# OpenResearchInstitute/opv-cxx-demod

Hardware: AMD Instinct MI355X
Metric: IQ Msamples/s demod+Viterbi (×real-time @2.168MSPS); BER vs ref (higher is better)
Workload: dtype f64; 1 GPU; configs[3]: 64 concurrent IQ streams/GPU x 1000 frames, -s semantics, amp 2000, f0 -2000..+2000 Hz across the 64 streams of a shard (SURVEY.md §8d C4: edge streams on the AFC clamp, outside the +/-1530 Hz search span), Eb/N0 16 dB; streams_per_gpu=64, parallelism=streams sharded 64/GPU, no data-path collective

## Files before the change

opv-cxx-demod_amd/csrc/k_frontend.hip:

```cpp
#include <hip/hip_runtime.h>
#include <math.h>

#include <type_traits>

#include "k_frontend_common.h"

namespace {

constexpr uint32_t kTile = OPV_TILE_SAMPLES;
constexpr uint32_t kRing = 2 * kTile;
constexpr uint32_t kRingBytes = kRing * 4;
constexpr uint32_t kGuardBytes = 16;
constexpr uint32_t kBack = 11;
constexpr uint32_t kAhead = 56;
static_assert((kRing & (kRing - 1)) == 0, "ring must be a power of two");

constexpr uint32_t kTabOff = kRingBytes + kGuardBytes;
static_assert(kTabOff % 16 == 0, "16-byte LDS alignment");
constexpr uint32_t kAtanQBytes = 1025 * 32;
constexpr uintptr_t kRbLdsBase = 16;
static_assert(kRbLdsBase + kTabOff + kAtanQBytes == OPV_RB_LDS_I16, "launch size of the int16-ring shape");

constexpr uint32_t kF64Ring = 2048;
constexpr uint32_t kF64RingBytes = kF64Ring * 32;
constexpr uint32_t kF64Chunk = 256;
constexpr uint32_t kF64TabOff = 0;
constexpr uint32_t kF64RingOff = kAtanQBytes;
constexpr uint32_t kF64FlagOff = kF64RingOff + kF64RingBytes;
constexpr uint32_t kF64WaitSpins = 1u << 22;
constexpr uint32_t kHelperSpins = 1u << 22;
static_assert(kRbLdsBase + kF64FlagOff + 16 == OPV_RB_LDS_F64, "launch size of the fp64-ring shape");
static_assert(kF64Ring % kF64Chunk == 0 && (kF64Ring & (kF64Ring - 1)) == 0, "chunks tile the power-of-two ring");

typedef double d2v __attribute__((ext_vector_type(2)));
typedef __attribute__((address_space(3))) unsigned char lbyte;
typedef __attribute__((address_space(3))) int lint;
typedef __attribute__((address_space(3))) double ldouble;
typedef __attribute__((address_space(3))) d2v ld2v;

__device__ inline double swap32_add(double a, double b) {
    auto lo = __builtin_amdgcn_permlane32_swap((unsigned)dlo(a), (unsigned)dlo(b), false, false);
    auto hi = __builtin_amdgcn_permlane32_swap((unsigned)dhi(a), (unsigned)dhi(b), false, false);
    return mkd((int)hi[0], (int)lo[0]) + mkd((int)hi[1], (int)lo[1]);
}
__device__ inline double swap16_add(double a, double b) {
    auto lo = __builtin_amdgcn_permlane16_swap((unsigned)dlo(a), (unsigned)dlo(b), false, false);
    auto hi = __builtin_amdgcn_permlane16_swap((unsigned)dhi(a), (unsigned)dhi(b), false, false);
    return mkd((int)hi[0], (int)lo[0]) + mkd((int)hi[1], (int)lo[1]);
}
template <int N>
__device__ inline double row_bcast(double old, double v) { return __builtin_amdgcn_update_dpp(old, v, 0x150 + N, 0xF, 0xF, false); }
__device__ inline uint32_t uni(uint32_t v) { return (uint32_t)__builtin_amdgcn_readfirstlane((int)v); }
__device__ inline bool uni_lt(double a, double b) { return __builtin_amdgcn_fcmp(a, b, 4 ) != 0ull; }
__device__ inline bool uni_eq(double a, double b) { return __builtin_amdgcn_fcmp(a, b, 1 ) != 0ull; }

struct TagFirst { static constexpr bool first = true, wide = true; };
struct TagSecond { static constexpr bool first = false, wide = true; };
struct TagSteady { static constexpr bool first = false, wide = false; };

struct SinCosK {
    double s0, s1, s2, s3;
    double c0, c1, c2, c3, c4;
};
#define OPV_EXPJ_ASM \
    "v_mul_f64 %[x], %[kfs], %[fo]\n\t" \
    "v_mul_f64 %[u], %[x], %[x]\n\t" \
    "v_fma_f64 %[r], %[c4], %[u], %[c3]\n\t" \
    "v_fma_f64 %[p], %[s3], %[u], %[s2]\n\t" \
    "v_fma_f64 %[r], %[r], %[u], %[c2]\n\t" \
    "v_fma_f64 %[p], %[p], %[u], %[s1]\n\t" \
    "v_fma_f64 %[r], %[r], %[u], %[c1]\n\t" \
    "v_fma_f64 %[p], %[p], %[u], %[s0]\n\t" \
    "v_fma_f64 %[r], %[r], %[u], %[c0]\n\t" \
    "v_mul_f64 %[t], %[x], %[u]\n\t" \
    "v_fma_f64 %[xc], %[r], %[u], 1.0\n\t" \
    "v_fma_f64 %[xs], %[t], %[p], %[x]"
__device__ inline void expj_small(double kfs, double fo, const SinCosK& k, double& xs, double& xc) {
    double x, u, p, r, t;
    asm(OPV_EXPJ_ASM
        : [x] "=&v"(x), [u] "=&v"(u), [p] "=&v"(p), [r] "=&v"(r), [t] "=&v"(t), [xs] "=&v"(xs), [xc] "=&v"(xc)
        : [kfs] "v"(kfs), [fo] "v"(fo), [s0] "v"(k.s0), [s1] "v"(k.s1), [s2] "v"(k.s2), [s3] "v"(k.s3),
          [c0] "v"(k.c0), [c1] "v"(k.c1), [c2] "v"(k.c2), [c3] "v"(k.c3), [c4] "v"(k.c4));
}
__device__ inline void expj_small_clamped(double kfs, double fo_raw, double fo_lo, double fo_hi, const SinCosK& k, double& fo,
                                          double& xs, double& xc) {
    double x, u, p, r, t;
    asm("v_max_f64 %[fo], %[raw], %[lo]\n\t"
        "v_min_f64 %[fo], %[fo], %[hi]\n\t" OPV_EXPJ_ASM
        : [fo] "=&v"(fo), [x] "=&v"(x), [u] "=&v"(u), [p] "=&v"(p), [r] "=&v"(r), [t] "=&v"(t), [xs] "=&v"(xs), [xc] "=&v"(xc)
        : [raw] "v"(fo_raw), [lo] "v"(fo_lo), [hi] "v"(fo_hi), [kfs] "v"(kfs), [s0] "v"(k.s0), [s1] "v"(k.s1), [s2] "v"(k.s2), [s3] "v"(k.s3),
          [c0] "v"(k.c0), [c1] "v"(k.c1), [c2] "v"(k.c2), [c3] "v"(k.c3), [c4] "v"(k.c4));
}
#undef OPV_EXPJ_ASM

}

#include "opv_atan2.h"

typedef __attribute__((address_space(3))) volatile uint32_t lds_flag;
__device__ inline lds_flag* f64_flags(lbyte* lds_all) {
    return reinterpret_cast<lds_flag*>(lds_all + kF64FlagOff);
}

__device__ void f64_ring_helper(const OpvStream& st, lbyte* lds_all) {
    const uint32_t lane = threadIdx.x & 63u;
    lds_flag* const fl = f64_flags(lds_all);
    const uint32_t n_avail = uni((uint32_t)st.n_avail), origin = uni((uint32_t)st.origin);
    const int* const iq = reinterpret_cast<const int*>(st.iq);
    uint32_t fill = ((origin >= kBack ? origin - kBack : 0u) / kF64Chunk) * kF64Chunk;
    const uint32_t fill_end = n_avail + kAhead + 2u;
    uint32_t spins = 0;
    while ((int)(fill - fill_end) < 0) {
        if (fl[2] != 0u) return;
        if ((int)(fl[0] + kF64Ring - fill - kF64Chunk) < 0) {
            if (++spins > kHelperSpins) return;
            __builtin_amdgcn_s_sleep(8);
            continue;
        }
        spins = 0;
        constexpr uint32_t kPerLane = kF64Chunk / 64u;
        const uint32_t n0 = fill + lane;
        int w[kPerLane], wn[kPerLane];
        if (fill + kF64Chunk < n_avail) {
#pragma unroll
            for (uint32_t k = 0; k < kPerLane; ++k) { w[k] = iq[n0 + 64u * k]; wn[k] = iq[n0 + 64u * k + 1u]; }
        } else {
#pragma unroll
            for (uint32_t k = 0; k < kPerLane; ++k) {
                const uint32_t n = n0 + 64u * k;
                w[k] = n < n_avail ? iq[n] : 0;
                wn[k] = n + 1u < n_avail ? iq[n + 1u] : 0;
            }
        }
#pragma unroll
        for (uint32_t k = 0; k < kPerLane; ++k) {
            const int xr = (int)(short)(w[k] & 0xFFFF), xi = w[k] >> 16;
            const int yr = (int)(short)(wn[k] & 0xFFFF) - xr, yi = (wn[k] >> 16) - xi;
            ld2v* e = reinterpret_cast<ld2v*>(lds_all + kF64RingOff + (((n0 + 64u * k) & (kF64Ring - 1u)) << 5));
            e[0] = d2v{(double)xr, (double)xi};
            e[1] = d2v{(double)yr, (double)yi};
        }
        __builtin_amdgcn_fence(__ATOMIC_RELEASE, "workgroup");
        fill += kF64Chunk;
        if (lane == 0u) fl[1] = fill;
    }
}

template <int WPB, bool F64 = false>
__device__ __forceinline__ void msk_frontend_body(OpvStream* __restrict__ streams, OpvGlobalCfg cfg, int n_streams,
                                                  lbyte* lds_all) {
    const int lane = threadIdx.x & 63;
    const int wave = WPB == 1 ? 0 : __builtin_amdgcn_readfirstlane((int)(threadIdx.x >> 6));
    const int sidx = (int)blockIdx.x * WPB + wave;
    const uint64_t dbg_t0 = __builtin_amdgcn_s_memtime(), dbg_r0 = __builtin_amdgcn_s_memrealtime();

    lbyte* const lds = lds_all + (F64 ? kF64RingOff : wave * kTabOff);
    const lbyte* ringb = lds;
    const ldouble* atab = reinterpret_cast<const ldouble*>(lds_all + (F64 ? kF64TabOff : WPB * kTabOff));
    if (sidx >= n_streams) return;
    OpvStream& st = streams[sidx];

    const int jsamp = (lane & 15) == 15 ? 50 : lane - (lane >> 4);
    const double kf = (double)(jsamp - 10);
    const double kfs = kf * kDeltaPerHz;
    double wr[15], wi[15];
    {
        const int row = lane >> 4, t = lane & 15, u = t & 7;
        const bool is_p = u >= 6, imag = t >= 8;
        const int gate = (u < 2 || is_p) ? 1 : ((u & 1) ? 2 : 0);
        const bool tone2 = is_p ? false : (u < 2 ? u == 1 : u >= 4);
#pragma unroll
        for (int n = 0; n < 15; ++n) {
            const int i = 15 * row + n - 10 * gate;
            double sn, cs;
            sincospi((double)i / 80.0, &sn, &cs);
            const bool in = i >= 0 && i < 40;
            const double a = in ? cs : 0.0, b = in ? -sn : 0.0;
            double r_, i_;
            if (is_p) { r_ = (t == 6) ? a : (t == 15 ? b : 0.0); i_ = (t == 7) ? b : (t == 14 ? a : 0.0); }
            else if (!imag) { r_ = a; i_ = tone2 ? -b : b; }
            else { r_ = tone2 ? b : -b; i_ = a; }
            wr[n] = r_; wi[n] = i_;
            asm volatile("" : "+v"(wr[n]), "+v"(wi[n]));
        }
    }
    SinCosK sck;
    sck.s0 = -0x1.5555555555412p-3; sck.s1 = 0x1.1111110f26395p-7; sck.s2 = -0x1.a019e48059d90p-13; sck.s3 = 0x1.7150a543fadc5p-19;
    sck.c0 = -0x1.0000000000000p-1; sck.c1 = 0x1.5555555555014p-5; sck.c2 = -0x1.6c16c16818f3fp-10;
    sck.c3 = 0x1.a019dfaa26924p-16; sck.c4 = -0x1.276f06eab6283p-22;
    double kc_tfmax = 0.1, kc_beta = 0.00001, kc_alpha = 0.005, kc_fomax = 2000.0, kc_eps = 1e-10;
    double kc_tiny = 1e-100;
    asm volatile("" : "+v"(kc_tiny));
    double kc_halfpi = 1.57079632679489661923, kc_32 = 32.0, kc_m1_32 = -1.0 / 32.0, kc_gain = st.afc_alpha * (kSymRate / kTwoPi);
    [[maybe_unused]] double kc_64 = 512.0, kc_m1_64 = -1.0 / 512.0, kc_magic = 6755399441055744.0 + 512.0;
    asm volatile("" : "+v"(kc_64), "+v"(kc_m1_64), "+v"(kc_magic));
    asm volatile("" : "+v"(kc_tfmax), "+v"(kc_beta), "+v"(kc_alpha), "+v"(kc_fomax), "+v"(kc_eps));
    asm volatile("" : "+v"(kc_halfpi), "+v"(kc_32), "+v"(kc_m1_32), "+v"(kc_gain));
    const double kc_nfomax = __builtin_canonicalize(-kc_fomax), kc_ntfmax = __builtin_canonicalize(-kc_tfmax);
    kc_fomax = __builtin_canonicalize(kc_fomax);
    kc_tfmax = __builtin_canonicalize(kc_tfmax);
    double sx = 1.0, nsg = 1.0;
    asm volatile("" : "+v"(sx), "+v"(nsg));

    double fo = st.freq_offset, tf = st.timing_freq, mu = st.mu;
    PrevSums qp{st.p1r, st.p1i, st.p2r, st.p2i, st.x40c, st.x40s}, qq{0, 0, 0, 0, 1, 0};
    double fo_sum = st.fo_sum;
    uint32_t origin = uni((uint32_t)st.origin);
    const uint32_t n_avail = uni((uint32_t)st.n_avail);
    uint64_t n_soft = st.n_soft, total_samples = st.total_samples;
    uint32_t n_chunks = uni(st.n_chunks);
    int tail_done = (int)uni((uint32_t)st.tail_done);
    const int eof = (int)uni((uint32_t)st.eof);
    int overflow = (int)uni((uint32_t)st.overflow), stalled = 0;
    uint32_t edge_ties = uni(st.edge_ties);
    const uint64_t cap_soft = st.cap_soft;
    if (cap_soft > (1ull << 28)) overflow = 1;
    uint64_t soft_keep = st.trk_next >= 24 ? st.trk_next - 24 : 0;
    if (st.trk_state != 0 && st.trk_anchor < soft_keep) soft_keep = st.trk_anchor;
    const uint32_t soft_bmask = (uint32_t)(cap_soft * 8u - 1u) & ~7u;
    gbyte* const soft_base = (gbyte*)(((uint64_t)uni((uint32_t)((uint64_t)st.soft >> 32)) << 32) | uni((uint32_t)(uint64_t)st.soft));
    const gbyte* iq_bytes = (const gbyte*)st.iq;
    const uint64_t n_bytes = (uint64_t)n_avail * 4u;

    auto glds16 = [&](const gbyte* gsrc, uint32_t lds_byte) {
        unsigned keep;
        asm volatile("s_mov_b32 %0, m0\n\ts_mov_b32 m0, %2\n\ts_nop 0\n\tglobal_load_lds_dwordx4 %1, off\n\ts_mov_b32 m0, %0"
                     : "=&s"(keep)
                     : "v"(gsrc), "s"(uni(lds_byte))
                     : "memory");
    };
    const uint32_t lds_base = uni((uint32_t)(uintptr_t)lds);
    auto issue_tile = [&](uint32_t t) {
        const uint64_t base = (uint64_t)t * OPV_TILE_BYTES;
        const uint32_t slot = (t & 1u) * OPV_TILE_BYTES;
#pragma unroll
        for (int r = 0; r < 8; ++r) {
            const uint32_t in_tile = (uint32_t)r * 1024u + (uint32_t)lane * 16u;
            const uint64_t off = base + in_tile;
            if (off + 16u <= n_bytes) glds16(iq_bytes + off, lds_base + slot + (uint32_t)r * 1024u);
            else if (off < n_bytes) {
                for (uint32_t j = 0; off + 4u * j < n_bytes; ++j)
                    *reinterpret_cast<lint*>(lds + slot + in_tile + 4u * j) = *reinterpret_cast<const __attribute__((address_space(1))) int*>(iq_bytes + off + 4u * j);
            }
        }
        if ((t & 1u) == 0u && lane == 0) {
            if (base + 16u <= n_bytes) glds16(iq_bytes + base, lds_base + kRingBytes);
            else
                for (uint32_t j = 0; base + 4u * j < n_bytes && j < 4u; ++j)
                    *reinterpret_cast<lint*>(lds + kRingBytes + 4u * j) = *reinterpret_cast<const __attribute__((address_space(1))) int*>(iq_bytes + base + 4u * j);
        }
    };
    uint32_t t_lo = (origin >= kBack ? origin - kBack : 0u) / kTile;
    if constexpr (!F64) {
        issue_tile(t_lo);
        issue_tile(t_lo + 1u);
        __builtin_amdgcn_s_waitcnt(0x0F70);
    }
    bool evt_issue = true;
    uint32_t next_evt = (t_lo + 1u) * kTile + kBack;
    [[maybe_unused]] lds_flag* const fl = f64_flags(lds_all);
    [[maybe_unused]] auto f64_wait = [&](uint32_t need) {
        uint32_t r = uni(fl[1]);
        for (uint32_t spins = 0; (int)(r - need) < 0;) {
            if (overflow != 0 || ++spins > kF64WaitSpins) { overflow = 2; break; }
            __builtin_amdgcn_s_sleep(1);
            r = uni(fl[1]);
        }
        return r;
    };

    for (;;) {
        const uint32_t remaining = n_avail - origin;
        uint32_t N;
        bool last = false;
        if (cfg.streaming) {
            if (remaining >= OPV_CHUNK) N = OPV_CHUNK;
            else if (eof && !tail_done && remaining > 0) { N = remaining; last = true; }
            else { if (eof) tail_done = 1; break; }
        } else {
            if (!eof || tail_done) break;
            N = n_avail;
            last = true;
        }
        if (overflow) break;
        if ((n_soft - soft_keep) + (uint64_t)(N / 38u + 2u) > cap_soft) { stalled = 1; break; }

        const double Nd = (double)N;
        double pos = mu;
        const uint32_t soft_off0 = ((uint32_t)n_soft * 8u) & soft_bmask;
        uint32_t soft_off = soft_off0;
        uint32_t soft_v = soft_off0;
        asm volatile("" : "+v"(soft_v));
        auto soft_advance = [&](uint32_t nsym) {
            soft_off = (soft_off + 8u * nsym) & soft_bmask;
            soft_v = soft_off;
            asm volatile("" : "+v"(soft_v));
        };
        const uint32_t ring_c = (origin << 5) & (kF64RingBytes - 1u);
        double fo_raw = fo;

        using NoAdvance = std::integral_constant<uint32_t, 0>;
        auto housekeeping = [&](double at, auto adv) {
            uint32_t bv = (uint32_t)at;
            asm("" : "+v"(bv));
            const uint32_t b = uni(bv);
            const uint32_t gb = origin + b;
            [[maybe_unused]] uint32_t ready_v = 0;
            if constexpr (F64) {
                if (lane == 0) fl[0] = gb >= kBack ? gb - kBack : 0u;
                ready_v = fl[1];
                __builtin_amdgcn_sched_barrier(0);
            }
            if constexpr (std::is_same_v<decltype(adv), uint32_t>) soft_advance(adv);
            int lim2 = (int)N - 52 - (int)b;
            uint32_t by_ring = ((soft_bmask + 8u - soft_off) >> 3) - 1u;
            if constexpr (F64) {
                asm volatile("" : "+s"(lim2), "+s"(by_ring));
                __builtin_amdgcn_sched_barrier(0);
                uint32_t ready = uni(ready_v);
                if (__builtin_expect((int)(ready - gb) < (int)(kAhead + 2u), 0)) ready = f64_wait(gb + kAhead + 2u);
                asm volatile("" ::: "memory");
                next_evt = ready - kAhead;
            }
            while (!F64 && gb >= next_evt) {
                if (evt_issue) {
                    issue_tile(t_lo + 2u);
                    ++t_lo;
                    evt_issue = false;
                    next_evt = (t_lo + 1u) * kTile - kAhead;
                } else {
                    __builtin_amdgcn_s_waitcnt(0x0F70);
                    evt_issue = true;
                    next_evt = (t_lo + 1u) * kTile + kBack;
                }
            }
            const int lim1 = (int)(next_evt - gb) - 2;
            int lim = lim1 < lim2 ? lim1 : lim2;
            if (lim < 0) lim = 0;
            const uint32_t by_samples = ((uint32_t)lim * 1560u) >> 16;
            return by_samples < by_ring ? by_samples : by_ring;
        };

        int w0 = 0, w1 = 0;
        [[maybe_unused]] d2v x0{0.0, 0.0}, dx{0.0, 0.0};
        double f = 0.0;
        uint32_t tap_byte = 0;
        auto fetch_addr = [&](double at, bool clamp0) {
            double p = at + kf;
            if (clamp0) p = fmax(p, 0.0);
            const int idx = (int)p;
            f = __builtin_amdgcn_fract(p);
            if constexpr (F64) asm("v_mad_legacy_u16 %0, %1, 32, %2" : "+v"(tap_byte) : "v"(idx), "s"(ring_c));
            else tap_byte = (((uint32_t)idx + origin) << 2) & (kRingBytes - 4u);
        };
        auto fetch_read = [&]() {
            if constexpr (F64) {
                const ld2v* tap = reinterpret_cast<const ld2v*>(ringb + tap_byte);
                x0 = tap[0];
                dx = tap[1];
            } else {
                const lint* tap = reinterpret_cast<const lint*>(ringb + tap_byte);
                w0 = tap[0];
                w1 = tap[1];
            }
        };
        auto fetch = [&](double at, bool clamp0) {
            fetch_addr(at, clamp0);
            fetch_read();
        };

        auto symbol_r = [&](auto tag, auto slot, PrevSums& cur, const PrevSums& prv) {
            constexpr bool kFirst = decltype(tag)::first;
            constexpr bool kWide = decltype(tag)::wide;
            constexpr uint32_t kSlot = decltype(slot)::value;
            double xs, xc;
            if constexpr (kWide) {
                if (__builtin_expect(uni_lt(2000.0, fabs(fo)), 0)) sincos(kfs * fo, &xs, &xc);
                else expj_small(kfs, fo, sck, xs, xc);
            } else {
                expj_small_clamped(kfs, fo_raw, kc_nfomax, kc_fomax, sck, fo, xs, xc);
            }
            __builtin_amdgcn_sched_barrier(0);
            double lr, li;
            if constexpr (F64) {
                lr = fma(f, dx.x, x0.x);
                li = fma(f, dx.y, x0.y);
            } else {
                const int s0r = (int)(short)(w0 & 0xFFFF), s0i = w0 >> 16;
                const int d_r = (int)(short)(w1 & 0xFFFF) - s0r, d_i = (w1 >> 16) - s0i;
                lr = fma(f, (double)d_r, (double)s0r);
                li = fma(f, (double)d_i, (double)s0i);
            }
            const double zr = fma(lr, xc, li * xs);
            const double zi = fma(li, xc, -(lr * xs));
            __builtin_amdgcn_sched_barrier(0);

            double acc0, acc1, v, t;
#define OPV_RB(N) "v_fmac_f64_dpp %[a0], %[zr], %[r" #N "] row_newbcast:" #N " row_mask:0xf bank_mask:0xf\n\t" \
                  "v_fmac_f64_dpp %[a1], %[zi], %[i" #N "] row_newbcast:" #N " row_mask:0xf bank_mask:0xf\n\t"
            asm("v_mov_b64 %[a0], 0\n\tv_mov_b64 %[a1], 0\n\t" OPV_RB(0) OPV_RB(1) OPV_RB(2) OPV_RB(3) OPV_RB(4) OPV_RB(5) OPV_RB(6) OPV_RB(7)
                OPV_RB(8) OPV_RB(9) OPV_RB(10) OPV_RB(11) OPV_RB(12) OPV_RB(13) OPV_RB(14)
                "v_add_f64 %[v], %[a0], %[a1]\n\t"
                "v_mov_b64 %[t], %[v]"
                : [a0] "=&v"(acc0), [a1] "=&v"(acc1), [v] "=&v"(v), [t] "=&v"(t)
                : [zr] "v"(zr), [zi] "v"(zi), [r0] "v"(wr[0]), [i0] "v"(wi[0]), [r1] "v"(wr[1]), [i1] "v"(wi[1]), [r2] "v"(wr[2]), [i2] "v"(wi[2]),
                  [r3] "v"(wr[3]), [i3] "v"(wi[3]), [r4] "v"(wr[4]), [i4] "v"(wi[4]), [r5] "v"(wr[5]), [i5] "v"(wi[5]),
                  [r6] "v"(wr[6]), [i6] "v"(wi[6]), [r7] "v"(wr[7]), [i7] "v"(wi[7]),
                  [r8] "v"(wr[8]), [i8] "v"(wi[8]), [r9] "v"(wr[9]), [i9] "v"(wi[9]), [r10] "v"(wr[10]), [i10] "v"(wi[10]),
                  [r11] "v"(wr[11]), [i11] "v"(wi[11]), [r12] "v"(wr[12]), [i12] "v"(wi[12]), [r13] "v"(wr[13]), [i13] "v"(wi[13]),
                  [r14] "v"(wr[14]), [i14] "v"(wi[14]));
#undef OPV_RB
            __builtin_amdgcn_sched_barrier(0);
            cur.x40c = row_bcast<15>(lr, xc);
            cur.x40s = row_bcast<15>(li, xs);
            __builtin_amdgcn_sched_barrier(0);
            v = swap32_add(v, t);
            asm("v_mov_b64 %0, %1" : "=v"(t) : "v"(v));
            __builtin_amdgcn_sched_barrier(0);
            v = swap16_add(v, t);
            __builtin_amdgcn_sched_barrier(0);
            double fo_sum_next = fo_sum + fo;
            asm volatile("" : "+v"(fo_sum_next));
            const double sq = v * v;
            __builtin_amdgcn_sched_barrier(0);
            const double shv = mkd(__builtin_amdgcn_mov_dpp(dhi(v), 0x128, 0xF, 0xF, true), __builtin_amdgcn_mov_dpp(dlo(v), 0x128, 0xF, 0xF, true));
            const double en = fma(shv, shv, sq);
            __builtin_amdgcn_sched_barrier(0);
            const double P1o = row_bcast<6>(zr, v), P2o = row_bcast<7>(zi, v);
            __builtin_amdgcn_sched_barrier(0);
            const double en1 = row_bcast<0>(acc0, en), en2 = row_bcast<1>(acc1, en);
            const double soft = en2 - en1;
            __builtin_amdgcn_sched_barrier(0);
            double P3o, P4o;
            int sel_lo, sel_hi;
            asm("v_cmp_gt_f64 vcc, 0, %[soft]\n\t"
                "v_mov_b64_dpp %[p3], %[v] row_newbcast:14 row_mask:0xf bank_mask:0xf\n\t"
                "v_mov_b64_dpp %[p4], %[v] row_newbcast:15 row_mask:0xf bank_mask:0xf\n\t"
                "v_cndmask_b32_dpp %[sl], %[el], %[el], vcc row_shl:2 row_mask:0xf bank_mask:0xf bound_ctrl:1\n\t"
                "v_cndmask_b32_dpp %[sh], %[eh], %[eh], vcc row_shl:2 row_mask:0xf bank_mask:0xf bound_ctrl:1"
                : [p3] "=&v"(P3o), [p4] "=&v"(P4o), [sl] "=&v"(sel_lo), [sh] "=&v"(sel_hi)
                : [soft] "v"(soft), [v] "v"(v), [el] "v"(dlo(en)), [eh] "v"(dhi(en))
                : "vcc");
            const double seln = mkd(sel_hi, sel_lo);
            __builtin_amdgcn_sched_barrier(0);
            nsg = mkd((dhi(soft) & (int)0x80000000) | (dhi(nsg) & 0x7fffffff), dlo(nsg));
            asm volatile("" : "+v"(nsg));
            const double sg = -nsg;
            __builtin_amdgcn_sched_barrier(0);

            [[maybe_unused]] double pd = 0.0, cx = 0, cy = 0, sum = 1.0, dif = 0, dm_ = 1.0, ee, el;
            [[maybe_unused]] uint64_t zmask = 0;
            if constexpr (!kFirst) {
                const double dr = fma(sg, P2o, P1o), di = fma(-sg, P4o, P3o);
                const double prs = fma(sg, prv.a, prv.b), pis = fma(sg, prv.c, -prv.d);
                const double ar = fma(dr, prs, di * pis), ai = fma(di, prs, -(dr * pis));
                cy = fma(ar, prv.x40c, ai * prv.x40s);
                cx = fma(ar, prv.x40s, -(ai * prv.x40c));
                __builtin_amdgcn_sched_barrier(0);
                ee = row_bcast<2>(sq, seln); el = row_bcast<3>(shv, seln);
                __builtin_amdgcn_sched_barrier(0);
                sx = mkd((dhi(cx) & (int)0x80000000) | (dhi(sx) & 0x7fffffff), dlo(sx));
                asm volatile("" : "+v"(sx));
                sum = fabs(cx) + fabs(cy); dif = fabs(cy) - fabs(cx);
                dm_ = sum + kc_tiny;
                if constexpr (WPB == 1) {
                    zmask = __builtin_amdgcn_fcmp(sum, 0.0, 1 );
                    asm volatile("" : "+s"(zmask));
                }
            } else {
                ee = row_bcast<2>(sq, seln); el = row_bcast<3>(shv, seln);
            }
            const double den = el + ee + kc_eps;

            double ted, h = 0;
            [[maybe_unused]] d2v c01{0, 0}, c23{0, 0};
            if constexpr (kFirst) {
                double y = __builtin_amdgcn_rcp(den);
                const double num = el - ee;
                y = fma(fma(-den, y, 1.0), y, y);
                y = fma(fma(-den, y, 1.0), y, y);
                ted = num * y;
                ted = fma(fma(-den, ted, num), y, ted);
            } else {
                const double dm = dm_;
                const double tt = den * dm;
                double y = __builtin_amdgcn_rcp(tt);
                const double num = el - ee;
                y = fma(fma(-tt, y, 1.0), y, y);
                const double iden = y * dm, idm = y * den;
                const double ratio = dif * idm;
                const double kt = fma(ratio, kc_64, kc_magic);
                h = ratio;
                const lbyte* rowb = reinterpret_cast<const lbyte*>(atab) + ((unsigned)dlo(kt) << 5);
                const ld2v* trow = reinterpret_cast<const ld2v*>(rowb);
                c23 = trow[1]; c01 = trow[0];
                ted = num * iden;
                ted = fma(fma(-den, ted, num), iden, ted);
            }
            __builtin_amdgcn_sched_barrier(0);
            tf = clampd(fma(kc_beta, ted, tf), kc_ntfmax, kc_tfmax);
            const double adj = fma(kc_alpha, ted, tf);
            pos += 40.0 + adj;
            fetch_addr(pos, false);
            __builtin_amdgcn_sched_barrier(0);
            fetch_read();
            __builtin_amdgcn_sched_barrier(0);
            *(gdouble*)(soft_base + soft_v + 8u * kSlot) = soft;
            if constexpr (!kFirst) {
                const double pd_off = fma(-sx, kc_halfpi, kc_halfpi);
                __builtin_amdgcn_sched_barrier(0);
                if constexpr (F64) __builtin_amdgcn_s_waitcnt(0xC27F);
                else __builtin_amdgcn_s_waitcnt(0xC17F);
                __builtin_amdgcn_sched_barrier(0);
                pd = fma(c23.y, h, c23.x);
                pd = fma(pd, h, c01.y);
                pd = fma(pd, h, c01.x);
                pd = fma(sx, pd, pd_off);
                pd = mkd((dhi(pd) & 0x7fffffff) | (dhi(cy) & (int)0x80000000), dlo(pd));
                if (__builtin_expect(WPB == 1 ? zmask != 0ull : uni_eq(sum, 0.0), 0)) {
                    const double dr = fma(sg, P2o, P1o), di = fma(-sg, P4o, P3o);
                    const double2 sp = silence_pd(dr, di, prv, soft < 0.0, fo_sum, n_soft + (((soft_v + 8u * kSlot - soft_off0) & soft_bmask) >> 3),
                                                  P1o, P2o, P3o, P4o);
                    pd = sp.x;
                    edge_ties += uni((uint32_t)sp.y);
                }
                fo_raw = fma(kc_gain, pd, fo);
            }
            fo_sum = fo_sum_next;
            cur.a = P1o; cur.b = P2o; cur.c = P3o; cur.d = P4o;
        };

        auto fo_settle = [&]() {
            asm("v_max_f64 %0, %1, %2\n\tv_min_f64 %0, %0, %3" : "=&v"(fo) : "v"(fo_raw), "v"(kc_nfomax), "v"(kc_fomax));
            fo_raw = fo;
        };
        using Slot0 = std::integral_constant<uint32_t, 0>;
        using Slot1 = std::integral_constant<uint32_t, 1>;
        using Slot2 = std::integral_constant<uint32_t, 2>;
        using Slot3 = std::integral_constant<uint32_t, 3>;
        auto sym = [&](auto tag, auto slot, PrevSums& cur, const PrevSums& prv) { symbol_r(tag, slot, cur, prv); };

        if (uni_lt(pos + 40.0 + 10.0, Nd)) {
            (void)housekeeping(pos, NoAdvance{});
            fetch(pos, true);
            sym(TagFirst{}, Slot0{}, qp, qp);
            soft_advance(1u);
            if (__builtin_expect(uni_lt(2000.0, fabs(fo)), 0) && uni_lt(pos + 40.0 + 10.0, Nd)) {
                (void)housekeeping(pos, NoAdvance{});
                fetch(pos, false);
                sym(TagSecond{}, Slot0{}, qq, qp);
                fo_settle();
                soft_advance(1u);
                qp = qq;
            }
            while (uni_lt(pos + 40.0 + 10.0, Nd)) {
                uint32_t more = uni(housekeeping(pos, NoAdvance{}));
                if (F64 && overflow != 0) break;
                fetch(pos, false);
                if constexpr (F64) asm volatile("; opv_symbol_loop_top\n\ts_nop 0\n\ts_nop 0\n\ts_nop 0\n\ts_nop 0\n\ts_nop 0\n\ts_nop 0");
                while (more >= 4u) {
                    for (uint32_t quads = more >> 2; quads != 0u; --quads) {
                        sym(TagSteady{}, Slot0{}, qq, qp);
                        sym(TagSteady{}, Slot1{}, qp, qq);
                        sym(TagSteady{}, Slot2{}, qq, qp);
                        sym(TagSteady{}, Slot3{}, qp, qq);
                        soft_v += 32u;
                    }
                    more = uni(housekeeping(pos, more & ~3u));
                }
                if (F64 && overflow != 0) { fo_settle(); break; }
                uint32_t pairs = more >> 1;
                const uint32_t batch = 2u * pairs + 1u;
                for (; pairs != 0u; --pairs) {
                    sym(TagSteady{}, Slot0{}, qq, qp);
                    sym(TagSteady{}, Slot1{}, qp, qq);
                    soft_v += 16u;
                }
                sym(TagSteady{}, Slot0{}, qq, qp);
                fo_settle();
                soft_advance(batch);
                qp = qq;
            }
        }

        const uint32_t nsym_call = ((soft_off - soft_off0) & soft_bmask) >> 3;
        const uint32_t used = uni((uint32_t)pos);
        mu = pos - (double)used;
        const uint32_t leftover = N - used;
        if (lane == 0) {
            double* c = st.chunk_log + 5 * (size_t)(n_chunks % st.cap_chunks);
            c[0] = fo;
            c[1] = tf; c[2] = mu; c[3] = (double)leftover; c[4] = (double)nsym_call;
        }
        ++n_chunks;
        n_soft += nsym_call;
        total_samples += N;
        origin += (leftover > 0u && leftover < N) ? used : N;
        if (last) { tail_done = 1; break; }
    }

    if constexpr (F64) {
        if (lane == 0) fl[2] = 1u;
    }
    if (lane == 0) {
        st.freq_offset = fo;
        st.p1r = qp.a; st.p1i = qp.b; st.p2r = qp.c; st.p2i = qp.d; st.x40c = qp.x40c; st.x40s = qp.x40s;
        st.fo_sum = fo_sum;
        st.edge_ties = edge_ties;
        st.timing_freq = tf; st.mu = mu;
        st.origin = origin; st.n_soft = n_soft; st.total_samples = total_samples;
        st.n_chunks = n_chunks; st.tail_done = tail_done; st.overflow = overflow;
        st.stalled = stalled;
        unsigned hw, xcc;
        asm volatile("s_getreg_b32 %0, hwreg(HW_REG_HW_ID)" : "=s"(hw));
        asm volatile("s_getreg_b32 %0, hwreg(HW_REG_XCC_ID)" : "=s"(xcc));
        st.dbg_hw_id = hw; st.dbg_xcc_id = xcc;
        st.dbg_cycles = __builtin_amdgcn_s_memtime() - dbg_t0;
        st.dbg_ticks = __builtin_amdgcn_s_memrealtime() - dbg_r0;
    }
}

template <int NT>
__device__ __forceinline__ void load_atan_table_q(lbyte* lds_tab) {
    ldouble* atab = reinterpret_cast<ldouble*>(lds_tab);
    for (int i = threadIdx.x; i < 1025 * 4; i += NT) atab[i] = (&kOpvAtanTabQ3R[0][0])[i];
}
extern "C" __global__ __launch_bounds__(128) void k_msk_frontend_rb(OpvStream* __restrict__ streams, OpvGlobalCfg cfg,
                                                                     int n_streams) {
    lbyte* const lds_dyn = reinterpret_cast<lbyte*>(kRbLdsBase);
    if (blockDim.x == 128) {
        load_atan_table_q<128>(lds_dyn + kF64TabOff);
        if (threadIdx.x == 0) {
            __attribute__((address_space(3))) uint32_t* const fl = reinterpret_cast<__attribute__((address_space(3))) uint32_t*>(lds_dyn + kF64FlagOff);
            fl[0] = 0u;
            fl[1] = 0u;
            fl[2] = 0u;
        }
        __syncthreads();
        if (__builtin_amdgcn_readfirstlane((int)(threadIdx.x >> 6)) != 0) {
            if ((int)blockIdx.x < n_streams) f64_ring_helper(streams[blockIdx.x], lds_dyn);
            return;
        }
        msk_frontend_body<1, true>(streams, cfg, n_streams, lds_dyn);
    } else {
        load_atan_table_q<64>(lds_dyn + kTabOff);
        __syncthreads();
        msk_frontend_body<1>(streams, cfg, n_streams, lds_dyn);
    }
}
extern "C" __global__ __launch_bounds__(256) void k_msk_frontend_rb_wg4(OpvStream* __restrict__ streams, OpvGlobalCfg cfg,
                                                                         int n_streams) {
    __shared__ __attribute__((aligned(16))) unsigned char lds_all[4 * kTabOff + kAtanQBytes];
    lbyte* const lds = (lbyte*)lds_all;
    load_atan_table_q<256>(lds + 4 * kTabOff);
    __syncthreads();
    msk_frontend_body<4>(streams, cfg, n_streams, lds);
}
```

opv-cxx-demod_amd/csrc/k_frontend_rows.h:

```cpp
#pragma once
#include "k_frontend_common.h"

namespace {

struct RowTone { double soft, nsg; };

struct RowStream {
    double fo, tf, mu, fo_sum;
    PrevSums pv;
    uint32_t origin, n_avail, n_chunks, edge_ties, soft_bmask, cap_chunks;
    uint64_t n_soft, total_samples, cap_soft, soft_keep, n_bytes;
    int tail_done, overflow, stalled, eof;
    gbyte* soft_base;
    const gbyte* iq_bytes;
    double* chunk_log;
    bool done, in_call, first, last;
    uint32_t N, soft_off, soft_off0;
    double Nd, pos;
    double held;
    uint32_t held_off;
    bool held_valid;

    __device__ __forceinline__ void load(const OpvStream& st, bool have) {
        fo = st.freq_offset; tf = st.timing_freq; mu = st.mu; fo_sum = st.fo_sum;
        pv = PrevSums{st.p1r, st.p1i, st.p2r, st.p2i, st.x40c, st.x40s};
        origin = (uint32_t)st.origin;
        n_avail = (uint32_t)st.n_avail;
        n_soft = st.n_soft; total_samples = st.total_samples;
        n_chunks = st.n_chunks;
        tail_done = st.tail_done; overflow = st.overflow; stalled = 0;
        edge_ties = st.edge_ties;
        eof = st.eof;
        cap_soft = st.cap_soft;
        if (cap_soft > (1ull << 28)) overflow = 1;
        soft_keep = st.trk_next >= 24 ? st.trk_next - 24 : 0;
        if (st.trk_state != 0 && st.trk_anchor < soft_keep) soft_keep = st.trk_anchor;
        soft_bmask = (uint32_t)(cap_soft * 8u - 1u) & ~7u;
        soft_base = (gbyte*)st.soft;
        iq_bytes = (const gbyte*)st.iq;
        n_bytes = (uint64_t)n_avail * 4u;
        chunk_log = st.chunk_log;
        cap_chunks = st.cap_chunks;
        done = !have; in_call = false; first = false; last = false;
        N = 0; soft_off = 0; soft_off0 = 0; Nd = 0.0; pos = 0.0;
        held = 0.0; held_off = 0; held_valid = false;
    }

    __device__ __forceinline__ void store(OpvStream& st, uint64_t dbg_t0, uint64_t dbg_r0) const {
        st.freq_offset = fo; st.timing_freq = tf; st.mu = mu;
        st.p1r = pv.a; st.p1i = pv.b; st.p2r = pv.c; st.p2i = pv.d; st.x40c = pv.x40c; st.x40s = pv.x40s;
        st.fo_sum = fo_sum;
        st.origin = origin; st.n_soft = n_soft; st.total_samples = total_samples;
        st.n_chunks = n_chunks; st.tail_done = tail_done; st.overflow = overflow;
        st.stalled = stalled; st.edge_ties = edge_ties;
        unsigned hw, xcc;
        asm volatile("s_getreg_b32 %0, hwreg(HW_REG_HW_ID)" : "=s"(hw));
        asm volatile("s_getreg_b32 %0, hwreg(HW_REG_XCC_ID)" : "=s"(xcc));
        st.dbg_hw_id = hw; st.dbg_xcc_id = xcc;
        st.dbg_cycles = __builtin_amdgcn_s_memtime() - dbg_t0;
        st.dbg_ticks = __builtin_amdgcn_s_memrealtime() - dbg_r0;
    }

    __device__ __forceinline__ void flush_soft() {
        if (held_valid) *(gdouble*)(soft_base + held_off) = held;
        held_valid = false;
    }

    __device__ __forceinline__ void begin_call(const OpvGlobalCfg& cfg) {
        const uint32_t remaining = n_avail - origin;
        bool go = true;
        last = false;
        if (cfg.streaming) {
            if (remaining >= OPV_CHUNK) N = OPV_CHUNK;
            else if (eof && !tail_done && remaining > 0) { N = remaining; last = true; }
            else { if (eof) tail_done = 1; go = false; }
        } else {
            if (!eof || tail_done) go = false;
            else { N = n_avail; last = true; }
        }
        if (go && overflow) go = false;
        if (go && (n_soft - soft_keep) + (uint64_t)(N / 38u + 2u) > cap_soft) { stalled = 1; go = false; }
        if (go) {
            in_call = true;
            first = true;
            Nd = (double)N;
            pos = mu;
            soft_off0 = ((uint32_t)n_soft * 8u) & soft_bmask;
            soft_off = soft_off0;
        } else {
            done = true;
        }
    }

    __device__ __forceinline__ bool has_symbol() const { return pos + 40.0 + 10.0 < Nd; }

    __device__ __forceinline__ void end_call(bool writer_lane) {
        const uint32_t nsym_call = ((soft_off - soft_off0) & soft_bmask) >> 3;
        const uint32_t used = (uint32_t)pos;
        mu = pos - (double)used;
        const uint32_t leftover = N - used;
        if (writer_lane) {
            double* c = chunk_log + 5 * (size_t)(n_chunks % cap_chunks);
            c[0] = fo; c[1] = tf; c[2] = mu; c[3] = (double)leftover; c[4] = (double)nsym_call;
        }
        ++n_chunks;
        n_soft += nsym_call;
        total_samples += N;
        origin += (leftover > 0u && leftover < N) ? used : N;
        in_call = false;
        if (last) { tail_done = 1; done = true; }
    }

    __device__ __forceinline__ int quota() const {
        int krow = 0x7fffffff;
        if (in_call) {
            krow = 0;
            const double room = Nd - 51.0 - pos;
            if (!first && !(fabs(fo) > 2000.0) && room > 0.0) krow = (int)(room * (1.0 / 42.0));
        }
        return krow;
    }

    static __device__ __forceinline__ RowTone tone(double P1o, double P2o, double P3o, double P4o) {
        const double s1r_ = P1o + P2o, s1i_ = P3o - P4o;
        const double s2r_ = P1o - P2o, s2i_ = P3o + P4o;
        const double en1 = fma(s1r_, s1r_, s1i_ * s1i_);
        const double en2 = fma(s2r_, s2r_, s2i_ * s2i_);
        const double soft = en2 - en1;
        const double nsg = mkd((dhi(soft) & (int)0x80000000) | 0x3ff00000, 0);
        return RowTone{soft, nsg};
    }

    template <bool kGeneric>
    __device__ __forceinline__ void finish_symbol(double P1o, double P2o, double P3o, double P4o, double soft, double sg,
                                                  double Ere, double Eim, double Lre, double Lim, double x40c, double x40s,
                                                  const double* atab, double kgain, bool keeps) {
        const double ee = fma(Ere, Ere, Eim * Eim), el = fma(Lre, Lre, Lim * Lim);
        const double num = el - ee, den = el + ee + 1e-10;
        const double dr = fma(sg, P2o, P1o), di = fma(-sg, P4o, P3o);
        const double prs = fma(sg, pv.a, pv.b), pis = fma(sg, pv.c, -pv.d);
        const double ar = fma(dr, prs, di * pis), ai = fma(di, prs, -(dr * pis));
        const double cy = fma(ar, pv.x40c, ai * pv.x40s);
        const double cx = fma(ar, pv.x40s, -(ai * pv.x40c));
        const double sum = fabs(cx) + fabs(cy), dif = fabs(cy) - fabs(cx);
        const double dm = sum + 1e-100;
        const double tt = den * dm;
        double y = __builtin_amdgcn_rcp(tt);
        y = fma(fma(-tt, y, 1.0), y, y);
        const double iden = y * dm, idm = y * den;
        const double ratio = dif * idm;
        const double kt = fma(ratio, 128.0, 6755399441055744.0 + 128.0);
        const double h = fma(kt - (6755399441055744.0 + 128.0), -1.0 / 128.0, ratio);
        const double2* trow = reinterpret_cast<const double2*>(atab + (unsigned)dlo(kt) * 6u);
        const double2 c45 = trow[2], c23 = trow[1], c01 = trow[0];
        __builtin_amdgcn_sched_barrier(0);
        double ted = num * iden;
        ted = fma(fma(-den, ted, num), iden, ted);
        tf = clampd(fma(0.00001, ted, tf), -0.1, 0.1);
        const double adj = fma(0.005, ted, tf);
        double pos_next = pos + (40.0 + adj);
        if (keeps) { held = soft; held_off = soft_off; held_valid = true; }
        asm volatile("" : "+v"(pos_next), "+v"(tf), "+v"(held));
        __builtin_amdgcn_sched_barrier(0);
        if (!kGeneric || !first) {
            double pd = fma(c45.y, h, c45.x);
            pd = fma(pd, h, c23.y);
            pd = fma(pd, h, c23.x);
            pd = fma(pd, h, c01.y);
            pd = fma(pd, h, c01.x);
            const double sx = mkd((dhi(cx) & (int)0x80000000) | 0x3ff00000, 0);
            pd = fma(sx, pd, fma(-sx, 1.57079632679489661923, 1.57079632679489661923));
            pd = mkd((dhi(pd) & 0x7fffffff) | (dhi(cy) & (int)0x80000000), dlo(pd));
            if (sum == 0.0) {
                const double2 sp = silence_pd(dr, di, pv, soft < 0.0, fo_sum,
                                              (uint32_t)n_soft + (((soft_off - soft_off0) & soft_bmask) >> 3),
                                              P1o, P2o, P3o, P4o);
                pd = sp.x;
                edge_ties += (uint32_t)sp.y;
            }
            const double fo_used = fo;
            fo = clampd(fma(kgain, pd, fo), -2000.0, 2000.0);
            fo_sum += fo_used;
        } else {
            fo_sum += fo;
        }
        soft_off = (soft_off + 8u) & soft_bmask;
        pv.a = P1o; pv.b = P2o; pv.c = P3o; pv.d = P4o; pv.x40c = x40c; pv.x40s = x40s;
        pos = pos_next;
        first = false;
    }
};

}
```

opv-cxx-demod_amd/csrc/k_sync_track.hip:

```cpp
#include <hip/hip_runtime.h>
#include <math.h>
#include <stdint.h>

#include "opv_device.h"

namespace {

struct Corr { double raw, norm; };

__device__ inline Corr window_corr(const double* __restrict__ soft, uint32_t mask, uint64_t last) {
    const uint32_t w0 = (uint32_t)(last - (OPV_SYNC_BITS - 1));
    double sum = 0.0, energy = 0.0;
#pragma unroll
    for (int i = 0; i < OPV_SYNC_BITS; ++i) {
        const double s = soft[(w0 + (uint32_t)i) & mask];
        const double pat = ((OPV_SYNC_WORD >> (OPV_SYNC_BITS - 1 - i)) & 1u) ? -1.0 : 1.0;
        sum += s * pat;
        energy += fabs(s);
    }
    Corr c;
    c.raw = sum;
    c.norm = energy < 100.0 ? 0.0 : sum / energy;
    return c;
}

}

extern "C" __global__ __launch_bounds__(64) void k_sync_track(OpvStream* __restrict__ streams) {
    OpvStream& st = streams[blockIdx.x];
    const int lane = threadIdx.x;
    const double* __restrict__ soft = st.soft;
    const uint32_t mask = (uint32_t)(st.cap_soft - 1);
    const uint64_t n = st.n_soft;

    int state = st.trk_state, collecting = st.trk_collecting, misses = st.trk_misses;
    uint64_t anchor = st.trk_anchor, next = st.trk_next;
    double quality = st.trk_quality;
    uint32_t n_frames = st.n_frames, n_events = st.n_events;
    int overflow = st.overflow;
    if (lane == 0) st.dec_from = n_frames;

    auto event = [&](int kind, int count, uint64_t sym, double corr, double raw) {
        if (lane == 0) {
            OpvEventRec& e = st.events[n_events % st.cap_events];
            e.kind = kind; e.count = count; e.sym_idx = sym; e.corr = corr; e.raw = raw;
        }
        ++n_events;
    };
    int sync_ok = st.trk_sync_ok, stalled = 0;
    auto frames_full = [&]() { return n_frames - st.frames_popped >= st.cap_frames; };
    auto release = [&](uint64_t at) {
        if (lane == 0) {
            OpvFrameRec& f = st.frec[n_frames % st.cap_frames];
            f.payload_sym = anchor + 1;
            f.release_sym = at;
            f.quality = quality;
            f.sync_ok = sync_ok;
            f.pad = 0;
            st.metrics[n_frames % st.cap_frames] = INT32_MIN;
        }
        ++n_frames;
        collecting = 0;
    };

    for (;;) {
        if (overflow) break;
        if (state == 0) {
            uint64_t pos = next < (OPV_SYNC_BITS - 1) ? (uint64_t)(OPV_SYNC_BITS - 1) : next;
            bool found = false;
            while (pos < n) {
                const uint64_t cand = pos + (uint64_t)lane;
                Corr c = {0.0, 0.0};
                bool ok = false;
                if (cand < n) {
                    c = window_corr(soft, mask, cand);
                    ok = (c.raw >= 5000.0) && (c.norm >= 0.85);
                }
                const unsigned long long m = __ballot(ok);
                if (m) {
                    const int first = __ffsll((long long)m) - 1;
                    const uint64_t s = pos + (uint64_t)first;
                    const double nrm = __shfl(c.norm, first, 64), raw = __shfl(c.raw, first, 64);
                    state = 1;
                    sync_ok = 1;
                    quality = nrm;
                    anchor = s;
                    collecting = 1;
                    event(1, 0, s, nrm, raw);
                    next = s + 1;
                    found = true;
                    break;
                }
                pos += 64;
            }
            if (!found) { next = n; break; }
        } else if (state == 1) {
            const uint64_t r = anchor + OPV_CODED;
            if (r >= n) break;
            if (frames_full()) { stalled = 2; break; }
            release(r);
            state = 2;
            misses = 0;
            event(2, (int)n_frames, r, 0.0, 0.0);
            next = r + 1;
        } else {
            if (collecting) {
                const uint64_t r = anchor + OPV_CODED;
                if (r >= n) break;
                if (frames_full()) { stalled = 2; break; }
                release(r);
                next = r + 1;
                continue;
            }
            const uint64_t c = anchor + OPV_FSYMS;
            if (c >= n) break;
            const Corr k = window_corr(soft, mask, c);
            next = c + 1;
            if (k.norm >= 0.70) {
                misses = 0;
                quality = k.norm;
                collecting = 1;
                sync_ok = 1;
                event(3, 0, c, k.norm, k.raw);
            } else {
                ++misses;
                event(4, misses, c, k.norm, k.raw);
                if (misses >= 5) {
                    state = 0;
                    collecting = 0;
                    event(5, 0, c, k.norm, k.raw);
                    continue;
                }
                quality = k.norm;
                collecting = 1;
                sync_ok = 0;
            }
            anchor = c;
        }
    }

    if (lane == 0) {
        st.trk_state = state; st.trk_collecting = collecting; st.trk_misses = misses;
        st.trk_anchor = anchor; st.trk_next = next; st.trk_quality = quality;
        st.n_frames = n_frames; st.n_events = n_events; st.trk_sync_ok = sync_ok;
        st.stalled |= stalled;
    }
}
```

opv-cxx-demod_amd/csrc/opv_capi.hip:

```cpp
#include <climits>
#include <cmath>
#include <cstdlib>
#include <cstring>
#include <new>
#include <string>

#include "opv_ctx.h"
#include "opv_offset_host.h"
#include "opv_stream_rules.h"

namespace {

thread_local std::string g_err;

constexpr uint64_t kScaleWaveMaxFrames = 4096;
constexpr int kFrontendWg4MinStreams = 512;
constexpr int kFrontendX16MinStreams = 8192;
constexpr int kFrontendX16Wg8MinStreams = 16384;
constexpr int kFrontendX4MinStreams = 2049;

__global__ void k_apply_inputs(OpvStream* streams, const StreamIn* in, int n) {
    const int i = blockIdx.x * blockDim.x + threadIdx.x;
    if (i < n) {
        if (in[i].dirty) {
            streams[i].iq = in[i].iq;
            streams[i].n_avail = in[i].n_avail;
            streams[i].eof = in[i].eof;
        }
        streams[i].frames_popped = in[i].frames_popped;
        streams[i].events_popped = in[i].events_popped;
    }
}

__global__ void k_collect_counts(const OpvStream* streams, int32_t* counts, int n, int* any_stalled) {
    const int i = blockIdx.x * blockDim.x + threadIdx.x;
    if (i < n) {
        counts[i] = (int32_t)streams[i].n_frames;
        if (streams[i].stalled) *(volatile int*)any_stalled = 1;
    }
}

__global__ void k_fill_i32(int32_t* p, int32_t v, size_t n) {
    for (size_t i = (size_t)blockIdx.x * blockDim.x + threadIdx.x; i < n; i += (size_t)gridDim.x * blockDim.x) p[i] = v;
}

}

int opv_int_fail(int code, const char* what, hipError_t e) {
    char buf[512];
    if (e != hipSuccess) snprintf(buf, sizeof buf, "%s: %s", what, hipGetErrorString(e));
    else snprintf(buf, sizeof buf, "%s", what);
    g_err = buf;
    return code;
}

extern "C" const char* opv_last_error(void) { return g_err.c_str(); }
extern "C" int opv_abi_version(void) { return OPV_ABI_VERSION; }

extern "C" int opv_create(opv_ctx** out, int n_streams, const opv_cfg* cfg) {
    if (!out || !cfg || n_streams <= 0 || cfg->max_samples == 0) return fail(OPV_EINVAL, "opv_create: bad arguments");
    if (cfg->max_samples >= (1ull << 31)) return fail(OPV_EINVAL, "opv_create: max_samples must be < 2^31");
    if ((cfg->have_init_offset && !std::isfinite(cfg->init_offset_hz)) || !std::isfinite(cfg->afc_alpha) || (cfg->coherent && !std::isfinite(cfg->pll_bw_hz)))
        return fail(OPV_EINVAL, "opv_create: init_offset_hz / afc_alpha / pll_bw_hz must be finite");
    int ndev = 0;
    if (hipGetDeviceCount(&ndev) != hipSuccess || ndev <= 0) return fail(OPV_ENODEV, "no HIP device visible");
    if (cfg->device < 0 || cfg->device >= ndev) return fail(OPV_ENODEV, "opv_cfg.device out of range");
    HIPCHK(hipSetDevice(cfg->device));
    hipDeviceProp_t prop;
    HIPCHK(hipGetDeviceProperties(&prop, cfg->device));
    if (std::strncmp(prop.gcnArchName, "gfx950", 6) != 0)
        return fail(OPV_ENODEV, "device is not gfx950 (MI355X); this library carries gfx950 code objects only");

    opv_ctx* c = new (std::nothrow) opv_ctx();
    if (!c) return fail(OPV_ENOMEM, "host allocation failed");
    c->n_streams = n_streams;
    c->cfg = *cfg;
    c->n_cu = prop.multiProcessorCount;
    c->hs.resize(n_streams);
    c->mirror.resize(n_streams);

    const uint64_t M = cfg->max_samples;
    c->cap_soft = 1;
    while (c->cap_soft < M / 38 + 4096) c->cap_soft <<= 1;
    c->cap_frames = (uint32_t)(M / (uint64_t)(OPV_FSYMS * 38) + 4);
    c->cap_events = 4 * c->cap_frames + 64;
    c->cap_chunks = (uint32_t)(M / 80000 + 4);

    auto cleanup = [&](int code) { opv_destroy(c); return code; };
#define HIPCHK_C(expr)                                                        \
    do {                                                                      \
        hipError_t _e = (expr);                                               \
        if (_e != hipSuccess) return cleanup(fail(_e == hipErrorOutOfMemory ? OPV_ENOMEM : OPV_EHIP, #expr, _e)); \
    } while (0)

    HIPCHK_C(hipStreamCreateWithFlags(&c->stream, hipStreamNonBlocking));
    {
        int least = 0, greatest = 0;
        if (hipDeviceGetStreamPriorityRange(&least, &greatest) != hipSuccess ||
            hipStreamCreateWithPriority(&c->copy_stream, hipStreamNonBlocking, greatest) != hipSuccess) {
            (void)hipGetLastError();
            c->copy_stream = nullptr;
            HIPCHK_C(hipStreamCreateWithFlags(&c->copy_stream, hipStreamNonBlocking));
        }
    }
    const size_t S = (size_t)n_streams;
    HIPCHK_C(hipHostMalloc(&c->h_in, sizeof(StreamIn) * S * opv_ctx::kInSlots, hipHostMallocDefault));
    for (auto& e : c->in_ev) HIPCHK_C(hipEventCreateWithFlags(&e, hipEventDisableTiming));
    HIPCHK_C(hipHostMalloc(&c->h_stall, sizeof(int) * opv_ctx::kInSlots, hipHostMallocDefault));
    for (int i = 0; i < opv_ctx::kInSlots; ++i) c->h_stall[i] = 0;
    HIPCHK_C(hipEventCreateWithFlags(&c->done_ev, hipEventDisableTiming));
    HIPCHK_C(hipMalloc(&c->d_streams, sizeof(OpvStream) * S));
    HIPCHK_C(hipMalloc(&c->d_in, sizeof(StreamIn) * S));
    HIPCHK_C(hipMalloc(&c->d_soft, sizeof(double) * c->cap_soft * S));
    HIPCHK_C(hipMalloc(&c->d_frec, sizeof(OpvFrameRec) * c->cap_frames * S));
    HIPCHK_C(hipMalloc(&c->d_events, sizeof(OpvEventRec) * c->cap_events * S));
    HIPCHK_C(hipMalloc(&c->d_chunks, sizeof(double) * 5 * c->cap_chunks * S));
    HIPCHK_C(hipMalloc(&c->d_frames, (size_t)OPV_FB * c->cap_frames * S));
    HIPCHK_C(hipMalloc(&c->d_metrics, sizeof(int32_t) * c->cap_frames * S));
    HIPCHK_C(hipMalloc(&c->d_fscale, sizeof(double) * c->cap_frames * S));
    HIPCHK_C(hipMalloc(&c->d_counts, sizeof(int32_t) * S));
    {
        std::vector<double> w((size_t)OPV_SPS * 2 * OPV_OFFS_TERMS);
        for (int i = 0; i < OPV_SPS; ++i) {
            const double u = (double)i - 19.5, cs = std::cos(M_PI * i / 80.0), sn = std::sin(M_PI * i / 80.0);
            double t = 1.0;
            for (int k = 0; k < OPV_OFFS_TERMS; ++k) {
                w[((size_t)i * 2 + 0) * OPV_OFFS_TERMS + k] = cs * t;
                w[((size_t)i * 2 + 1) * OPV_OFFS_TERMS + k] = sn * t;
                t = t * u / (double)(k + 1);
            }
        }
        HIPCHK_C(hipMalloc(&c->d_offs_wtab, sizeof(double) * w.size()));
        HIPCHK_C(hipMemcpy(c->d_offs_wtab, w.data(), sizeof(double) * w.size(), hipMemcpyHostToDevice));
    }
    c->host_ties = opv_offset_host_libm_matches_reference() && !std::getenv("OPV_OFFSET_DISTRUST_LIBM");
    c->tx_trust_libm = opv_tx_libm_flat_tops_as_assumed() && !std::getenv("OPV_TX_DISTRUST_LIBM");
    c->push_gather = !std::getenv("OPV_PUSH_NO_GATHER");
    if (const char* e = std::getenv("OPV_PUSH_GATHER_BLOCKS")) { const int v = atoi(e); if (v > 0) c->push_gather_blocks = (uint32_t)v; }
    c->rb_fp64_ring = !std::getenv("OPV_FRONTEND_INT16_RING");
    {
        hipFuncAttributes fa;
        HIPCHK_C(hipFuncGetAttributes(&fa, (const void*)k_msk_frontend_rb));
        if (fa.sharedSizeBytes != 0) return cleanup(fail(OPV_EHIP, "k_msk_frontend_rb was built with static LDS"));
    }
    if (c->rb_fp64_ring) HIPCHK_C(hipFuncSetAttribute((const void*)k_msk_frontend_rb, hipFuncAttributeMaxDynamicSharedMemorySize, OPV_RB_LDS_F64));
    if (c->host_ties) {
        HIPCHK_C(hipMalloc(&c->d_tie_list, sizeof(uint32_t) * (S + 1)));
        c->tie.slots = (uint32_t)(S < (size_t)OPV_TIE_SLOTS_MAX ? S : (size_t)OPV_TIE_SLOTS_MAX);
        if (hipHostMalloc((void**)&c->tie.stage, offsetof(OpvTieStage, slot) + sizeof(OpvTieSlot) * c->tie.slots, hipHostMallocDefault) != hipSuccess) {
            (void)hipGetLastError();
            c->tie.stage = nullptr;
            c->host_ties = false;
        } else {
            c->tie.stage->n = c->tie.stage->listed = c->tie.stage->beyond = 0;
        }
    }
    HIPCHK_C(hipMemsetAsync(c->d_frames, 0, (size_t)OPV_FB * c->cap_frames * S, c->stream));
    HIPCHK_C(hipMemsetAsync(c->d_counts, 0, sizeof(int32_t) * S, c->stream));
    k_fill_i32<<<256, 256, 0, c->stream>>>(c->d_metrics, INT32_MIN, (size_t)c->cap_frames * S);

    for (size_t i = 0; i < S; ++i) {
        OpvStream s;
        std::memset(&s, 0, sizeof s);
        s.soft = c->d_soft + c->cap_soft * i;
        s.cap_soft = c->cap_soft;
        s.frec = c->d_frec + (size_t)c->cap_frames * i;
        s.events = c->d_events + (size_t)c->cap_events * i;
        s.chunk_log = c->d_chunks + (size_t)5 * c->cap_chunks * i;
        s.frames = c->d_frames + (size_t)OPV_FB * c->cap_frames * i;
        s.metrics = c->d_metrics + (size_t)c->cap_frames * i;
        s.fscale = c->d_fscale + (size_t)c->cap_frames * i;
        s.cap_frames = c->cap_frames;
        s.cap_events = c->cap_events;
        s.cap_chunks = c->cap_chunks;
        s.freq_offset = (cfg->streaming && cfg->have_init_offset) ? cfg->init_offset_hz : 0.0;
        s.afc_alpha = cfg->afc_alpha;
        s.est_offset = NAN;
        s.x40c = 1.0;
        s.trk_state = OPV_HUNTING;
        c->mirror[i] = s;
    }
    c->initial = c->mirror;
    HIPCHK_C(hipMemcpyAsync(c->d_streams, c->mirror.data(), sizeof(OpvStream) * S, hipMemcpyHostToDevice, c->stream));
    HIPCHK_C(hipStreamSynchronize(c->stream));
    c->mirror_valid = true;
    *out = c;
    return OPV_OK;
#undef HIPCHK_C
}

extern "C" void opv_destroy(opv_ctx* c) {
    if (!c) return;
    (void)hipSetDevice(c->cfg.device);
    if (c->copy_stream) (void)hipStreamSynchronize(c->copy_stream);
    if (c->stream) (void)hipStreamSynchronize(c->stream);
    for (auto& e : c->in_ev)
        if (e) (void)hipEventDestroy(e);
    if (c->h_in) (void)hipHostFree(c->h_in);
    if (c->h_stall) (void)hipHostFree(c->h_stall);
    if (c->tie.stage) (void)hipHostFree(c->tie.stage);
    if (c->push_ev) (void)hipEventDestroy(c->push_ev);
    if (c->done_ev) (void)hipEventDestroy(c->done_ev);
    if (c->copy_stream) (void)hipStreamDestroy(c->copy_stream);
    for (auto& h : c->hs) { (void)hipFree(h.d_iq_owned); (void)hipFree(h.d_iq_alt); }
    for (auto& e : c->ev)
        if (e) (void)hipEventDestroy(e);
    void* ptrs[] = {c->d_streams, c->d_in, c->d_soft, c->d_frec, c->d_events, c->d_chunks, c->d_frames, c->d_metrics, c->d_fscale, c->d_counts, c->d_link, c->d_offs_wtab, c->d_tx_cnt, c->d_tx_list, c->d_tie_list};
    for (void* p : ptrs)
        if (p) (void)hipFree(p);
    if (c->stream) (void)hipStreamDestroy(c->stream);
    delete c;
}

static void tie_host_fn(void* p) {
    opv_ctx::TieWork* w = (opv_ctx::TieWork*)p;
    uint32_t n = w->stage->n;
    if (n > w->slots) n = w->slots;
    if (w->stage->beyond) w->left.fetch_add(w->stage->beyond, std::memory_order_relaxed);
    if (n == 0) return;
    opv_offset_decide_slots(w->stage->slot, n);
    w->decided.fetch_add(n, std::memory_order_relaxed);
}

extern "C" int opv_process(opv_ctx* c) {
    if (!c) return fail(OPV_EINVAL, "null context");
    HIPCHK(hipSetDevice(c->cfg.device));
    const int S = c->n_streams;
    const int slot = (int)(c->round_no % opv_ctx::kInSlots);
    if (c->round_no >= (unsigned)opv_ctx::kInSlots) HIPCHK(hipEventSynchronize(c->in_ev[slot]));
    StreamIn* in = c->h_in + (size_t)slot * S;
    uint64_t max_new = 0, max_tapped = 0;
    bool any = false;
    c->search_now.clear();
    for (int i = 0; i < S; ++i) {
        const HostStream& h = c->hs[i];
        in[i] = {h.d_iq, h.n_avail, h.eof, h.dirty ? 1 : 0, h.popped, h.events_popped};
        if (h.dirty) any = true;
        if (!h.search_seen && (c->cfg.streaming ? h.n_avail >= (uint64_t)OPV_CHUNK : h.eof != 0)) c->search_now.push_back(i);
        const uint64_t fresh = h.n_avail - h.last_round_avail;
        if (fresh > max_new) max_new = fresh;
        if (h.tap_fresh) any = true;
        if (h.tap_fresh > max_tapped) max_tapped = h.tap_fresh;
    }
    if (!any && c->maybe_stalled && c->round_no > 0 && hipEventQuery(c->done_ev) == hipSuccess)
        c->maybe_stalled = c->h_stall[(c->round_no - 1) % opv_ctx::kInSlots] != 0;
    if (!any && !c->maybe_stalled) return OPV_OK;
    uint64_t fr = max_new / (uint64_t)(OPV_FSYMS * 38);
    if (max_tapped / (uint64_t)OPV_FSYMS > fr) fr = max_tapped / (uint64_t)OPV_FSYMS;
    fr += 4;
    if (fr > c->cap_frames) fr = c->cap_frames;
    if (fr * (uint64_t)S > 0x7FFFFFFFull) return fail(OPV_EINVAL, "opv_process: streams x frames per round exceeds the grid limit");
    for (int i = 0; i < S; ++i) {
        HostStream& h = c->hs[i];
        h.last_round_avail = h.n_avail;
        h.dirty = false;
        h.tap_fresh = 0;
    }
    for (int i : c->search_now) c->hs[i].search_seen = true;
    c->mirror_valid = false;
    c->maybe_stalled = true;
    c->h_stall[slot] = 0;
    if (c->push_pending) HIPCHK(hipStreamWaitEvent(c->stream, c->push_ev, 0));
    HIPCHK(hipMemcpyAsync(c->d_in, in, sizeof(StreamIn) * S, hipMemcpyHostToDevice, c->stream));
    HIPCHK(hipEventRecord(c->in_ev[slot], c->stream));
    ++c->round_no;
    OpvGlobalCfg g{c->cfg.streaming, c->cfg.have_init_offset, c->cfg.init_offset_hz};
    k_apply_inputs<<<(S + 63) / 64, 64, 0, c->stream>>>(c->d_streams, c->d_in, S);
    const bool tm = c->timing;
    if (tm) HIPCHK(hipEventRecord(c->ev[0], c->stream));
    const size_t n_search = (c->cfg.streaming && c->cfg.have_init_offset) ? 0 : c->search_now.size();
    const bool host_ties = n_search != 0 && c->host_ties;
    if (host_ties) HIPCHK(hipMemsetAsync(c->d_tie_list, 0, sizeof(uint32_t), c->stream));
    k_offset_search<<<S, 256, 0, c->stream>>>(c->d_streams, g, c->d_offs_wtab, host_ties ? c->d_tie_list : nullptr);
    if (tm) HIPCHK(hipEventRecord(c->ev[1], c->stream));
    if (host_ties) {
        const uint32_t K = c->tie.slots;
        uint32_t passes = (uint32_t)((n_search + K - 1) / K);
        if (passes > OPV_TIE_PASSES_MAX) passes = OPV_TIE_PASSES_MAX;
        for (uint32_t p = 0; p < passes; ++p) {
            k_tie_collect<<<K, 256, 0, c->stream>>>(c->d_streams, c->d_tie_list, p, K, p + 1 == passes ? 1u : 0u, c->tie.stage);
            if (hipLaunchHostFunc(c->stream, tie_host_fn, &c->tie) != hipSuccess) {
                (void)hipGetLastError();
                c->host_ties = false;
                break;
            }
            k_tie_apply<<<K, 192, 0, c->stream>>>(c->d_streams, c->tie.stage, K, S);
        }
    }
    if (tm) HIPCHK(hipEventRecord(c->ev[2], c->stream));
    const bool x4 = c->frontend == 4 || (c->frontend == 0 && S >= kFrontendX4MinStreams);
    if (c->cfg.coherent && !c->cfg.streaming) {
        const double wn = c->cfg.pll_bw_hz * 2.0 * M_PI, zeta = 0.707, fsym = 2168000.0 / 40.0;
        c->last_frontend = "k_coherent_frontend";
        k_coherent_frontend<<<S, 64, 0, c->stream>>>(c->d_streams, 2.0 * zeta * wn / fsym, wn * wn / (fsym * fsym));
    }
    else if (c->frontend == 16 || (c->frontend == 0 && S > kFrontendX16MinStreams)) {
        if (S > kFrontendX16Wg8MinStreams) { c->last_frontend = "k_msk_frontend_x16_wg8"; k_msk_frontend_x16_wg8<<<(S + 127) / 128, 512, 0, c->stream>>>(c->d_streams, g, S); }
        else if (S > 16) { c->last_frontend = "k_msk_frontend_x16_wg4"; k_msk_frontend_x16_wg4<<<(S + 63) / 64, 256, 0, c->stream>>>(c->d_streams, g, S); }
        else { c->last_frontend = "k_msk_frontend_x16"; k_msk_frontend_x16<<<1, 64, 0, c->stream>>>(c->d_streams, g, S); }
    }
    else if (x4) {
        c->last_frontend = "k_msk_frontend_x4_wg4";
        k_msk_frontend_x4_wg4<<<(S + 15) / 16, 256, 0, c->stream>>>(c->d_streams, g, S);
    }
    else if (S > kFrontendWg4MinStreams) {
        c->last_frontend = "k_msk_frontend_rb_wg4";
        k_msk_frontend_rb_wg4<<<(S + 3) / 4, 256, 0, c->stream>>>(c->d_streams, g, S);
    } else if (c->rb_fp64_ring && S <= c->n_cu) {
        c->last_frontend = "k_msk_frontend_rb";
        k_msk_frontend_rb<<<S, 128, OPV_RB_LDS_F64, c->stream>>>(c->d_streams, g, S);
    } else {
        c->last_frontend = "k_msk_frontend_rb";
        k_msk_frontend_rb<<<S, 64, OPV_RB_LDS_I16, c->stream>>>(c->d_streams, g, S);
    }
    if (tm) { HIPCHK(hipEventRecord(c->ev[3], c->stream)); HIPCHK(hipEventRecord(c->ev[4], c->stream)); }
    k_sync_track<<<S, 64, 0, c->stream>>>(c->d_streams);
    if (tm) { HIPCHK(hipEventRecord(c->ev[5], c->stream)); HIPCHK(hipEventRecord(c->ev[6], c->stream)); }
    if (fr * (uint64_t)S <= kScaleWaveMaxFrames) k_frame_scale_wave<<<(unsigned)(fr * (uint64_t)S), 64, 0, c->stream>>>(c->d_streams, (uint32_t)fr);
    else k_frame_scale<<<(unsigned)((fr * (uint64_t)S + 63) / 64), 64, 0, c->stream>>>(c->d_streams, (uint32_t)fr, (uint32_t)S);
    k_frame_decode<<<(unsigned)(((fr + 1) / 2) * (uint64_t)S), 64, 0, c->stream>>>(c->d_streams, (uint32_t)((fr + 1) / 2));
    if (tm) { HIPCHK(hipEventRecord(c->ev[7], c->stream)); c->timing_valid = true; }
    link_launch(c, fr);
    k_collect_counts<<<(S + 63) / 64, 64, 0, c->stream>>>(c->d_streams, c->d_counts, S, c->h_stall + slot);
    HIPCHK(hipEventRecord(c->done_ev, c->stream));
    HIPCHK(hipGetLastError());
    return OPV_OK;
}

extern "C" int opv_set_frontend(opv_ctx* c, int streams_per_wave) {
    if (!c) return fail(OPV_EINVAL, "null context");
    if (streams_per_wave != 0 && streams_per_wave != 1 && streams_per_wave != 4 && streams_per_wave != 16)
        return fail(OPV_EINVAL, "opv_set_frontend: 0 (automatic), 1, 4 or 16 streams per wave");
    c->frontend = streams_per_wave;
    return OPV_OK;
}

extern "C" const char* opv_frontend_kernel(opv_ctx* c) { return c ? c->last_frontend : ""; }

extern "C" int opv_sync(opv_ctx* c) {
    if (!c) return fail(OPV_EINVAL, "null context");
    HIPCHK(hipStreamSynchronize(c->stream));
    return OPV_OK;
}

extern "C" int opv_reset_stream(opv_ctx* c, int s) {
    if (!c) return fail(OPV_EINVAL, "null context");
    if (s != -1) { if (int r = check_stream(c, s)) return r; }
    if (int r = settle_pushes(c)) return r;
    HIPCHK(hipStreamSynchronize(c->stream));
    const int lo = (s == -1) ? 0 : s, hi = (s == -1) ? c->n_streams : s + 1;
    for (int i = lo; i < hi; ++i) c->hs[i] = reset_host_stream(c->hs[i]);
    HIPCHK(hipMemcpyAsync(c->d_streams + lo, &c->initial[lo], sizeof(OpvStream) * (hi - lo), hipMemcpyHostToDevice, c->stream));
    k_fill_i32<<<256, 256, 0, c->stream>>>(c->d_metrics + (size_t)c->cap_frames * lo, INT32_MIN,
                                          (size_t)c->cap_frames * (hi - lo));
    if (int r = link_clear(c, lo, hi)) return r;
    HIPCHK(hipStreamSynchronize(c->stream));
    c->mirror_valid = false;
    return OPV_OK;
}

extern "C" int opv_enable_timing(opv_ctx* c, int enable) {
    if (!c) return fail(OPV_EINVAL, "null context");
    HIPCHK(hipSetDevice(c->cfg.device));
    if (enable)
        for (auto& e : c->ev)
            if (!e) HIPCHK(hipEventCreate(&e));
    c->timing = enable != 0;
    c->timing_valid = false;
    return OPV_OK;
}

extern "C" int opv_kernel_times(opv_ctx* c, float ms[4]) {
    if (!c || !ms) return fail(OPV_EINVAL, "null argument");
    if (!c->timing_valid) return fail(OPV_ESTATE, "no timed opv_process yet (opv_enable_timing first)");
    HIPCHK(hipStreamSynchronize(c->stream));
    for (int k = 0; k < 4; ++k) HIPCHK(hipEventElapsedTime(&ms[k], c->ev[2 * k], c->ev[2 * k + 1]));
    return OPV_OK;
}

static int ring_to_host(opv_ctx* c, void* dst, const void* d_ring, uint32_t first, uint32_t n, uint32_t cap, size_t elem) {
    const RingRuns r = ring_runs(first, n, cap);
    bool have = false;
    if (int r = c->ensure_pools(&have)) return r;
    if (have) {
        if (const void* h_ring = c->host_view(d_ring)) {
            std::memcpy(dst, (const char*)h_ring + r.p0 * elem, r.run0 * elem);
            if (r.run1) std::memcpy((char*)dst + r.run0 * elem, h_ring, r.run1 * elem);
            return OPV_OK;
        }
    }
    HIPCHK(hipMemcpy(dst, (const char*)d_ring + r.p0 * elem, r.run0 * elem, hipMemcpyDeviceToHost));
    if (r.run1) HIPCHK(hipMemcpy((char*)dst + r.run0 * elem, d_ring, r.run1 * elem, hipMemcpyDeviceToHost));
    return OPV_OK;
}

extern "C" long opv_pop_frames(opv_ctx* c, int s, uint8_t* out, size_t cap, opv_frame_meta* meta) {
    if (int r = check_stream(c, s)) return r;
    if (int r = c->refresh()) return r;
    const OpvStream& st = c->mirror[s];
    if (st.overflow == 2) return fail(OPV_EHIP, "front-end: the two wavefronts of a stream lost each other (hand-over timed out)");
    if (st.overflow) return fail(OPV_EINVAL, "opv_cfg.max_samples too large for the soft-symbol ring (internal limit 2^28 symbols)");
    HostStream& h = c->hs[s];
    const uint32_t nf = st.n_frames;
    if (h.popped >= nf || cap == 0) return 0;
    size_t w = 0;
    uint32_t f = h.popped;
    std::vector<int32_t> met;
    std::vector<OpvFrameRec> rec;
    std::vector<uint8_t> fr;
    while (f < nf && w < cap) {
        uint32_t n = nf - f;
        if (n > cap - w) n = (uint32_t)(cap - w);
        if (n > st.cap_frames) n = st.cap_frames;
        met.resize(n);
        rec.resize(n);
        fr.resize((size_t)n * OPV_FB);
        if (int r = ring_to_host(c, met.data(), st.metrics, f, n, st.cap_frames, sizeof(int32_t))) return r;
        if (int r = ring_to_host(c, rec.data(), st.frec, f, n, st.cap_frames, sizeof(OpvFrameRec))) return r;
        if (int r = ring_to_host(c, fr.data(), st.frames, f, n, st.cap_frames, OPV_FB)) return r;
        bool stop = false;
        for (uint32_t k = 0; k < n; ++k, ++f) {
            if (met[k] == INT32_MIN) { stop = true; break; }
            if (met[k] < 0) continue;
            if (out) std::memcpy(out + w * OPV_FB, fr.data() + (size_t)k * OPV_FB, OPV_FB);
            if (meta) {
                meta[w].viterbi_metric = met[k];
                meta[w].sync_ok = rec[k].sync_ok;
                meta[w].sync_quality = rec[k].quality;
                meta[w].release_symbol = rec[k].release_sym;
                meta[w].payload_symbol = rec[k].payload_sym;
            }
            ++h.decoded;
            if (met[k] == 0) ++h.perfect;
            ++w;
        }
        if (stop) break;
    }
    h.popped = f;
    return (long)w;
}

extern "C" long opv_pop_events(opv_ctx* c, int s, opv_event* out, size_t cap) {
    if (int r = check_stream(c, s)) return r;
    if (int r = c->refresh()) return r;
    const OpvStream& st = c->mirror[s];
    HostStream& h = c->hs[s];
    const uint32_t ne = st.n_events;
    if (ne - h.events_popped > st.cap_events) {
        h.events_dropped += (ne - h.events_popped) - st.cap_events;
        h.events_popped = ne - st.cap_events;
    }
    if (h.events_popped >= ne || cap == 0 || !out) return 0;
    uint32_t n = ne - h.events_popped;
    if (n > cap) n = (uint32_t)cap;
    static_assert(sizeof(opv_event) == sizeof(OpvEventRec), "event layouts must match");
    if (int r = ring_to_host(c, out, st.events, h.events_popped, n, st.cap_events, sizeof(OpvEventRec))) return r;
    h.events_popped += n;
    return (long)n;
}

extern "C" int opv_get_state(opv_ctx* c, int s, opv_stream_state* out) {
    if (int r = check_stream(c, s)) return r;
    if (!out) return fail(OPV_EINVAL, "null out");
    if (int r = c->refresh()) return r;
    const OpvStream& st = c->mirror[s];
    std::memset(out, 0, sizeof *out);
    out->freq_offset_hz = st.freq_offset;
    out->timing_freq = st.timing_freq;
    out->est_offset_hz = st.est_offset;
    out->mu = st.mu;
    out->total_symbols = st.n_soft;
    out->total_samples = st.total_samples;
    out->chunk_origin = st.origin + st.iq_base;
    out->sync_state = st.trk_state;
    out->frames_released = (int32_t)st.n_frames;
    out->n_chunks = (int32_t)st.n_chunks;
    out->flushed = st.tail_done;
    const HostStream& h = c->hs[s];
    out->frames_decoded = h.decoded;
    out->frames_perfect = h.perfect;
    out->events_dropped = h.events_dropped;
    if (st.n_events - h.events_popped > st.cap_events) out->events_dropped += (st.n_events - h.events_popped) - st.cap_events;
    out->edge_ties = st.edge_ties;
    out->offset_ties = (int32_t)st.est_ties;
    out->stalled = st.stalled;
    if (st.n_frames > h.popped) {
        uint32_t n = st.n_frames - h.popped;
        if (n > st.cap_frames) n = st.cap_frames;
        std::vector<int32_t> met(n);
        if (int r = ring_to_host(c, met.data(), st.metrics, h.popped, n, st.cap_frames, sizeof(int32_t))) return r;
        for (int32_t m : met)
            if (m >= 0) { out->frames_decoded++; if (m == 0) out->frames_perfect++; }
    }
    return st.overflow ? fail(OPV_EINVAL, "opv_cfg.max_samples too large for the soft-symbol ring") : OPV_OK;
}

extern "C" int opv_device_frames(opv_ctx* c, const uint8_t** d_frames, const int32_t** d_metrics,
                                 const int32_t** d_counts, size_t* frame_capacity) {
    if (!c) return fail(OPV_EINVAL, "null context");
    if (d_frames) *d_frames = c->d_frames;
    if (d_metrics) *d_metrics = c->d_metrics;
    if (d_counts) *d_counts = c->d_counts;
    if (frame_capacity) *frame_capacity = c->cap_frames;
    return OPV_OK;
}

extern "C" void* opv_hip_stream(opv_ctx* c) { return c ? (void*)c->stream : nullptr; }

extern "C" long opv_tap_soft(opv_ctx* c, int s, uint64_t first, double* out, size_t cap) {
    if (int r = check_stream(c, s)) return r;
    if (int r = c->refresh()) return r;
    const OpvStream& st = c->mirror[s];
    if ((st.n_soft > st.cap_soft && first < st.n_soft - st.cap_soft) || (first < c->hs[s].soft_floor && first < st.n_soft))
        return fail(OPV_EINVAL, "soft symbols that old have been overwritten (the log is a ring)");
    if (first >= st.n_soft || cap == 0 || !out) return 0;
    uint64_t n = st.n_soft - first;
    if (n > cap) n = cap;
    const RingRuns r = ring_runs(first, n, st.cap_soft);
    HIPCHK(hipMemcpy(out, st.soft + r.p0, sizeof(double) * r.run0, hipMemcpyDeviceToHost));
    if (r.run1) HIPCHK(hipMemcpy(out + r.run0, st.soft, sizeof(double) * r.run1, hipMemcpyDeviceToHost));
    return (long)n;
}

extern "C" int opv_tap_push_soft(opv_ctx* c, int s, const double* soft, size_t n) {
    if (int r = check_stream(c, s)) return r;
    if (!soft || n == 0) return fail(OPV_EINVAL, "opv_tap_push_soft: null pointer or no symbols");
    HostStream& h = c->hs[s];
    if (h.iq_seen || h.attached || h.n_avail) return fail(OPV_ESTATE, "opv_tap_push_soft: the stream has received IQ (reset it first)");
    if (h.eof) return fail(OPV_ESTATE, "opv_tap_push_soft: the stream has been flushed (reset it first)");
    if (int r = settle_pushes(c)) return r;
    if (int r = c->refresh()) return r;
    OpvStream& st = c->mirror[s];
    if (st.overflow) return fail(OPV_ESTATE, "opv_tap_push_soft: the stream is in an error state (opv_pop_frames reports it)");
    if (n > st.cap_soft || (st.n_soft - soft_keep(st)) + n > st.cap_soft)
        return fail(OPV_ECAPACITY, "opv_tap_push_soft: the soft-symbol ring has no room (unread symbols + this push do not fit; "
                                   "call opv_process / opv_pop_frames between pushes)");
    const RingRuns r = ring_runs(st.n_soft, n, st.cap_soft);
    HIPCHK(hipMemcpyAsync(st.soft + r.p0, soft, sizeof(double) * r.run0, hipMemcpyHostToDevice, c->stream));
    if (r.run1) HIPCHK(hipMemcpyAsync(st.soft, soft + r.run0, sizeof(double) * r.run1, hipMemcpyHostToDevice, c->stream));
    st.n_soft += n;
    HIPCHK(hipMemcpyAsync(&c->d_streams[s].n_soft, &st.n_soft, sizeof st.n_soft, hipMemcpyHostToDevice, c->stream));
    HIPCHK(hipStreamSynchronize(c->stream));
    h.soft_tapped = true;
    h.tap_fresh += n;
    return OPV_OK;
}

extern "C" long opv_tap_chunks(opv_ctx* c, int s, uint32_t first, double* out5, size_t cap) {
    if (int r = check_stream(c, s)) return r;
    if (int r = c->refresh()) return r;
    const OpvStream& st = c->mirror[s];
    if (first >= st.n_chunks || cap == 0 || !out5) return 0;
    if (st.n_chunks - first > st.cap_chunks || first < c->hs[s].chunk_floor) return fail(OPV_EINVAL, "chunk log entries already overwritten (ring)");
    uint32_t n = st.n_chunks - first;
    if (n > cap) n = (uint32_t)cap;
    const RingRuns r = ring_runs(first, n, st.cap_chunks);
    HIPCHK(hipMemcpy(out5, st.chunk_log + 5 * r.p0, sizeof(double) * 5 * r.run0, hipMemcpyDeviceToHost));
    if (r.run1) HIPCHK(hipMemcpy(out5 + 5 * r.run0, st.chunk_log, sizeof(double) * 5 * r.run1, hipMemcpyDeviceToHost));
    return (long)n;
}

extern "C" int opv_tap_offset_energies(opv_ctx* c, int s, double* out134) {
    if (int r = check_stream(c, s)) return r;
    if (!out134) return fail(OPV_EINVAL, "null out");
    if (int r = c->refresh()) return r;
    std::memcpy(out134, c->mirror[s].energies, sizeof(double) * 134);
    return OPV_OK;
}

extern "C" int opv_offset_ties_on_host(opv_ctx* c) { return c && c->host_ties ? 1 : 0; }
extern "C" uint64_t opv_offset_ties_decided_on_host(opv_ctx* c) { return c ? c->tie.decided.load(std::memory_order_relaxed) : 0; }
extern "C" uint64_t opv_offset_ties_left_to_device(opv_ctx* c) { return c ? c->tie.left.load(std::memory_order_relaxed) : 0; }

extern "C" int opv_tap_wave_info(opv_ctx* c, int s, uint64_t out[4]) {
    if (int r = check_stream(c, s)) return r;
    if (!out) return fail(OPV_EINVAL, "null out");
    if (int r = c->refresh()) return r;
    const OpvStream& st = c->mirror[s];
    out[0] = st.dbg_hw_id; out[1] = st.dbg_xcc_id; out[2] = st.dbg_cycles; out[3] = st.dbg_ticks;
    return OPV_OK;
}

extern "C" int opv_tap_occupancy(opv_ctx* c, int out[6]) {
    if (!c || !out) return fail(OPV_EINVAL, "null argument");
    HIPCHK(hipSetDevice(c->cfg.device));
    const struct { const void* k; int threads; size_t lds; } ks[6] = {
        {(const void*)k_msk_frontend_rb, 64, OPV_RB_LDS_I16}, {(const void*)k_msk_frontend_rb_wg4, 256, 0}, {(const void*)k_msk_frontend_x16_wg4, 256, 0},
        {(const void*)k_msk_frontend_x4_wg4, 256, 0}, {(const void*)k_frame_decode, 64, 0}, {(const void*)k_frame_scale, 64, 0}};
    for (int i = 0; i < 6; ++i) HIPCHK(hipOccupancyMaxActiveBlocksPerMultiprocessor(&out[i], ks[i].k, ks[i].threads, ks[i].lds));
    return OPV_OK;
}

extern "C" int opv_decode_payloads(opv_ctx* c, const double* soft, size_t n, uint8_t* out, int32_t* metrics,
                                   int8_t* q, int8_t* deint, uint8_t* bits) {
    if (!c || !soft || !out || !metrics) return fail(OPV_EINVAL, "null argument");
    if (n == 0) return OPV_OK;
    HIPCHK(hipSetDevice(c->cfg.device));
    double* d_soft = nullptr;
    uint8_t* d_out = nullptr;
    int32_t* d_met = nullptr;
    int8_t *d_q = nullptr, *d_d = nullptr;
    uint8_t* d_b = nullptr;
    double* d_scale = nullptr;
    int rc = OPV_OK;
    auto chk = [&](hipError_t e, const char* w) { if (e != hipSuccess && rc == OPV_OK) rc = fail(OPV_EHIP, w, e); };
    chk(hipMalloc(&d_soft, sizeof(double) * OPV_CODED * n), "hipMalloc soft");
    chk(hipMalloc(&d_out, (size_t)OPV_FB * n), "hipMalloc out");
    chk(hipMalloc(&d_met, sizeof(int32_t) * n), "hipMalloc metrics");
    chk(hipMalloc(&d_scale, sizeof(double) * n), "hipMalloc scales");
    if (q) chk(hipMalloc(&d_q, (size_t)OPV_CODED * n), "hipMalloc q");
    if (deint) chk(hipMalloc(&d_d, (size_t)OPV_CODED * n), "hipMalloc deint");
    if (bits) chk(hipMalloc(&d_b, (size_t)OPV_FBITS * n), "hipMalloc bits");
    if (rc == OPV_OK) {
        chk(hipMemcpyAsync(d_soft, soft, sizeof(double) * OPV_CODED * n, hipMemcpyHostToDevice, c->stream), "H2D soft");
        chk(hipMemsetAsync(d_out, 0, (size_t)OPV_FB * n, c->stream), "memset");
        k_payload_scale<<<(unsigned)((n + 63) / 64), 64, 0, c->stream>>>(d_soft, (uint32_t)n, d_scale);
        k_decode_payloads<<<(unsigned)((n + 1) / 2), 64, 0, c->stream>>>(d_soft, (uint32_t)n, d_scale, d_out, d_met, d_q, d_d, d_b);
        chk(hipGetLastError(), "k_decode_payloads launch");
        chk(hipMemcpyAsync(out, d_out, (size_t)OPV_FB * n, hipMemcpyDeviceToHost, c->stream), "D2H out");
        chk(hipMemcpyAsync(metrics, d_met, sizeof(int32_t) * n, hipMemcpyDeviceToHost, c->stream), "D2H metrics");
        if (q) chk(hipMemcpyAsync(q, d_q, (size_t)OPV_CODED * n, hipMemcpyDeviceToHost, c->stream), "D2H q");
        if (deint) chk(hipMemcpyAsync(deint, d_d, (size_t)OPV_CODED * n, hipMemcpyDeviceToHost, c->stream), "D2H deint");
        if (bits) chk(hipMemcpyAsync(bits, d_b, (size_t)OPV_FBITS * n, hipMemcpyDeviceToHost, c->stream), "D2H bits");
        chk(hipStreamSynchronize(c->stream), "sync");
    }
    void* ptrs[] = {d_soft, d_out, d_met, d_q, d_d, d_b, d_scale};
    for (void* p : ptrs) if (p) (void)hipFree(p);
    return rc;
}
```

opv-cxx-demod_amd/csrc/opv_ctx.h:

```cpp
#pragma once
#include <hip/hip_runtime.h>

#include <atomic>
#include <cstdio>
#include <initializer_list>
#include <vector>

#include "../../include/opv_demod.h"
#include "opv_device.h"
#include "opv_wb_internal.h"

extern "C" __global__ void k_offset_search(OpvStream*, OpvGlobalCfg, const double*, uint32_t*);
extern "C" __global__ void k_tie_collect(const OpvStream*, const uint32_t*, uint32_t, uint32_t, uint32_t, OpvTieStage*);
extern "C" __global__ void k_tie_apply(OpvStream*, const OpvTieStage*, uint32_t, int);
extern "C" __global__ void k_msk_frontend_rb(OpvStream*, OpvGlobalCfg, int);
extern "C" __global__ void k_msk_frontend_rb_wg4(OpvStream*, OpvGlobalCfg, int);
extern "C" __global__ void k_msk_frontend_x4_wg4(OpvStream*, OpvGlobalCfg, int);
extern "C" __global__ void k_msk_frontend_x16(OpvStream*, OpvGlobalCfg, int);
extern "C" __global__ void k_msk_frontend_x16_wg4(OpvStream*, OpvGlobalCfg, int);
extern "C" __global__ void k_msk_frontend_x16_wg8(OpvStream*, OpvGlobalCfg, int);
extern "C" __global__ void k_coherent_frontend(OpvStream*, double, double);
extern "C" __global__ void k_sync_track(OpvStream*);
extern "C" __global__ void k_frame_scale(OpvStream*, uint32_t, uint32_t);
extern "C" __global__ void k_frame_scale_wave(OpvStream*, uint32_t);
extern "C" __global__ void k_frame_decode(OpvStream*, uint32_t);
extern "C" __global__ void k_payload_scale(const double*, uint32_t, double*);
extern "C" __global__ void k_decode_payloads(const double*, uint32_t, const double*, uint8_t*, int32_t*, int8_t*, int8_t*, uint8_t*);
extern "C" __global__ void k_frame_link(OpvStream*, opv_link*, uint32_t, uint32_t);
extern "C" __global__ void k_link_payloads(const double*, uint32_t, const double*, const uint8_t*, const int32_t*, opv_link*);
extern "C" __global__ void k_stream_pack(const OpvMove*, uint32_t);
extern "C" __global__ void k_stream_unpack(OpvStream*, int32_t*, const OpvUnpackItem*, uint32_t, const OpvMove*, uint32_t);
extern "C" __global__ void k_channel(const int4*, int4*, uint64_t, double, double, double, uint64_t);
extern "C" __global__ void k_resample_clock(const int*, uint64_t, int*, uint64_t, double);
extern "C" __global__ void k_tx_encode(const uint8_t*, uint32_t, uint8_t*, uint8_t*);
extern "C" __global__ void k_tx_scan_frames(uint8_t*, uint32_t);
extern "C" __global__ void k_tx_expand_phases(const double2*, uint32_t, uint64_t, uint64_t, double2*);
extern "C" __global__ void k_tx_modulate(const uint8_t*, const uint8_t*, const double2*, uint64_t, uint64_t, int*, uint32_t*, uint64_t*, uint32_t, uint64_t, uint64_t, const uint8_t*);
struct OpvTxbEntry;
struct OpvTxbAmb;
extern "C" __global__ void k_txb_encode(const OpvTxbEntry*, uint32_t, uint32_t, uint8_t*, uint8_t*);
extern "C" __global__ void k_txb_scan(const OpvTxbEntry*, uint32_t, uint8_t*, uint8_t*);
extern "C" __global__ void k_txb_phases(const OpvTxbEntry*, uint32_t, uint32_t, const double2*, double2*);
extern "C" __global__ void k_txb_modulate(const OpvTxbEntry*, uint32_t, const uint8_t*, const uint8_t*, const double2*, uint32_t*, OpvTxbAmb*, uint32_t, uint64_t, uint64_t, const uint8_t*);

inline int fail(int code, const char* what, hipError_t e = hipSuccess) { return opv_int_fail(code, what, e); }

#define HIPCHK(expr)                                              \
    do {                                                          \
        hipError_t _e = (expr);                                   \
        if (_e != hipSuccess) return fail(OPV_EHIP, #expr, _e);   \
    } while (0)

inline int alloc_failed(hipError_t e, const char* what, const char* oom) {
    if (!oom) return fail(OPV_EHIP, what, e);
    (void)hipGetLastError();
    return fail(OPV_ENOMEM, oom);
}

template <class T, bool kPinned = false>
struct GrowBuf {
    T* p = nullptr;
    size_t cap = 0;
    int grow(size_t need, size_t new_cap, std::initializer_list<hipStream_t> wait_for, const char* oom = nullptr) {
        if (cap >= need) return OPV_OK;
        for (hipStream_t s : wait_for) HIPCHK(hipStreamSynchronize(s));
        if (p) HIPCHK(kPinned ? hipHostFree(p) : hipFree(p));
        p = nullptr;
        cap = 0;
        const hipError_t e = kPinned ? hipHostMalloc((void**)&p, new_cap, hipHostMallocDefault) : hipMalloc((void**)&p, new_cap);
        if (e != hipSuccess) { p = nullptr; return alloc_failed(e, kPinned ? "hipHostMalloc" : "hipMalloc", oom); }
        cap = new_cap;
        return OPV_OK;
    }
    ~GrowBuf() { if (p) (void)(kPinned ? hipHostFree(p) : hipFree(p)); }
};

struct StreamIn {
    const int16_t* iq;
    uint64_t n_avail;
    int32_t eof;
    int32_t dirty;
    uint32_t frames_popped, events_popped;
};

struct HostStream {
    int16_t* d_iq_owned = nullptr;
    int16_t* d_iq_alt = nullptr;
    size_t iq_cap = 0;
    const int16_t* d_iq = nullptr;
    uint64_t n_avail = 0;
    int eof = 0;
    bool dirty = false;
    bool attached = false;
    bool search_seen = false;
    uint64_t last_round_avail = 0;
    uint32_t popped = 0;
    uint32_t events_popped = 0;
    uint32_t events_dropped = 0;
    int32_t decoded = 0, perfect = 0;
    uint64_t soft_floor = 0;
    uint32_t chunk_floor = 0;
    bool iq_seen = false;
    bool soft_tapped = false;
    uint64_t tap_fresh = 0;
};

inline HostStream reset_host_stream(const HostStream& h) {
    HostStream n;
    n.d_iq = n.d_iq_owned = h.d_iq_owned;
    n.d_iq_alt = h.d_iq_alt;
    n.iq_cap = h.iq_cap;
    return n;
}

struct opv_ctx {
    int n_streams = 0;
    opv_cfg cfg{};
    hipStream_t stream = nullptr;
    hipStream_t copy_stream = nullptr;
    OpvStream* d_streams = nullptr;
    StreamIn* d_in = nullptr;
    static constexpr int kInSlots = 4;
    StreamIn* h_in = nullptr;
    hipEvent_t in_ev[kInSlots] = {};
    int* h_stall = nullptr;
    hipEvent_t done_ev = nullptr;
    unsigned round_no = 0;
    std::vector<OpvStream> mirror;
    std::vector<OpvStream> initial;
    std::vector<HostStream> hs;
    double* d_soft = nullptr;
    OpvFrameRec* d_frec = nullptr;
    OpvEventRec* d_events = nullptr;
    double* d_chunks = nullptr;
    uint8_t* d_frames = nullptr;
    int32_t* d_metrics = nullptr;
    double* d_fscale = nullptr;
    int32_t* d_counts = nullptr;
    opv_link* d_link = nullptr;
    bool link_on = false;
    double* d_offs_wtab = nullptr;
    uint32_t* d_tie_list = nullptr;
    bool host_ties = false;
    bool tx_trust_libm = false;
    bool push_gather = true;
    uint32_t push_gather_blocks = 32;
    bool rb_fp64_ring = true;
    int n_cu = 0;
    struct TieWork {
        OpvTieStage* stage = nullptr;
        uint32_t slots = 0;
        std::atomic<uint64_t> decided{0};
        std::atomic<uint64_t> left{0};
    } tie;
    std::vector<int> search_now;
    GrowBuf<void, true> bulk_tab;
    bool push_pending = false;
    hipEvent_t push_ev = nullptr;
    OpvWbTie wb;
    GrowBuf<char> mig;
    GrowBuf<char, true> mig_tab;
    uint64_t cap_soft = 0;
    uint32_t cap_frames = 0, cap_events = 0, cap_chunks = 0;
    bool mirror_valid = false;
    bool maybe_stalled = false;
    GrowBuf<double> tx_ckpt;
    size_t tx_ckpt_have = 0;
    GrowBuf<double> tx_phases;
    size_t tx_phases_have = 0;
    GrowBuf<uint8_t> tx_scratch;
    uint32_t* d_tx_cnt = nullptr;
    uint64_t* d_tx_list = nullptr;
    GrowBuf<uint8_t> tx_flat;
    uint64_t tx_flat_lo = ~0ull, tx_flat_hi = ~0ull, tx_flat_have = 0;
    const char* last_frontend = "";
    int frontend = 0;
    bool timing = false;
    bool timing_valid = false;
    hipEvent_t ev[8] = {};

    static constexpr size_t kPoolMirrorMax = 64u << 20;
    std::vector<uint8_t> m_frames;
    std::vector<int32_t> m_metrics;
    std::vector<OpvFrameRec> m_frec;
    std::vector<OpvEventRec> m_events;
    unsigned mirror_epoch = 0, pools_epoch = ~0u;
    std::vector<opv_link> m_link;
    unsigned link_epoch = ~0u;

    int refresh() {
        if (mirror_valid) return OPV_OK;
        HIPCHK(hipSetDevice(cfg.device));
        HIPCHK(hipStreamSynchronize(stream));
        HIPCHK(hipMemcpy(mirror.data(), d_streams, sizeof(OpvStream) * n_streams, hipMemcpyDeviceToHost));
        mirror_valid = true;
        ++mirror_epoch;
        maybe_stalled = false;
        for (const OpvStream& m : mirror) maybe_stalled |= m.stalled != 0;
        return OPV_OK;
    }
    size_t pool_bytes() const {
        const size_t S = (size_t)n_streams;
        return S * ((size_t)cap_frames * (OPV_FB + sizeof(int32_t) + sizeof(OpvFrameRec)) + (size_t)cap_events * sizeof(OpvEventRec));
    }
    int ensure_pools(bool* have) {
        *have = false;
        if (pool_bytes() > kPoolMirrorMax) return OPV_OK;
        if (pools_epoch != mirror_epoch) {
            const size_t S = (size_t)n_streams;
            m_frames.resize((size_t)OPV_FB * cap_frames * S);
            m_metrics.resize((size_t)cap_frames * S);
            m_frec.resize((size_t)cap_frames * S);
            m_events.resize((size_t)cap_events * S);
            HIPCHK(hipMemcpy(m_frames.data(), d_frames, m_frames.size(), hipMemcpyDeviceToHost));
            HIPCHK(hipMemcpy(m_metrics.data(), d_metrics, m_metrics.size() * sizeof(int32_t), hipMemcpyDeviceToHost));
            HIPCHK(hipMemcpy(m_frec.data(), d_frec, m_frec.size() * sizeof(OpvFrameRec), hipMemcpyDeviceToHost));
            HIPCHK(hipMemcpy(m_events.data(), d_events, m_events.size() * sizeof(OpvEventRec), hipMemcpyDeviceToHost));
            pools_epoch = mirror_epoch;
        }
        *have = true;
        return OPV_OK;
    }
    const void* host_view(const void* d) const {
        auto in = [&](const void* base, size_t bytes) { return (const char*)d >= (const char*)base && (const char*)d < (const char*)base + bytes; };
        if (in(d_frames, m_frames.size())) return m_frames.data() + ((const char*)d - (const char*)d_frames);
        if (in(d_metrics, m_metrics.size() * sizeof(int32_t))) return (const char*)m_metrics.data() + ((const char*)d - (const char*)d_metrics);
        if (in(d_frec, m_frec.size() * sizeof(OpvFrameRec))) return (const char*)m_frec.data() + ((const char*)d - (const char*)d_frec);
        if (in(d_events, m_events.size() * sizeof(OpvEventRec))) return (const char*)m_events.data() + ((const char*)d - (const char*)d_events);
        return nullptr;
    }
};

inline int check_stream(opv_ctx* c, int s) {
    if (!c) return fail(OPV_EINVAL, "null context");
    if (s < 0 || s >= c->n_streams) return fail(OPV_EINVAL, "stream index out of range");
    return OPV_OK;
}

inline int settle_pushes(opv_ctx* c) {
    HIPCHK(hipSetDevice(c->cfg.device));
    if (c->push_pending) {
        HIPCHK(hipStreamSynchronize(c->copy_stream));
        c->push_pending = false;
    }
    return OPV_OK;
}

void link_launch(opv_ctx* c, uint64_t fr);
int link_clear(opv_ctx* c, int lo, int hi);
bool opv_tx_libm_flat_tops_as_assumed();
int opv_tx_prepare_run(opv_ctx* c, size_t nsym);
int ensure_iq_buffer(opv_ctx* c, HostStream& h, int which, const char* oom = nullptr);
```

opv-cxx-demod_amd/csrc/opv_device.h:

```cpp
#pragma once
#include <stdint.h>

#define OPV_SPS 40
#define OPV_SYNC_BITS 24
#define OPV_FB 134
#define OPV_FBITS 1072
#define OPV_CODED 2144
#define OPV_FSYMS 2168
#define OPV_CHUNK 86720
#define OPV_SYNC_WORD 0x02B8DBu

#define OPV_OFFS_TERMS 10

#define OPV_TILE_SAMPLES 2048
#define OPV_TILE_BYTES (OPV_TILE_SAMPLES * 4)
#define OPV_RB_LDS_I16 (16 + 2 * OPV_TILE_BYTES + 16 + 1025 * 32)
#define OPV_RB_LDS_F64 (16 + 1025 * 32 + 2048 * 32 + 16)

struct OpvFrameRec {
    uint64_t payload_sym;
    uint64_t release_sym;
    double quality;
    int32_t sync_ok;
    int32_t pad;
};

struct OpvEventRec {
    int32_t kind;
    int32_t count;
    uint64_t sym_idx;
    double corr;
    double raw;
};

struct OpvStream {
    const int16_t* iq;
    uint64_t n_avail;
    int32_t eof;
    int32_t pad0;
    double* soft;
    uint64_t cap_soft;
    uint64_t iq_base;
    uint32_t frames_popped, events_popped;
    OpvFrameRec* frec;
    OpvEventRec* events;
    double* chunk_log;
    uint8_t* frames;
    int32_t* metrics;
    double* fscale;
    uint32_t cap_frames, cap_events, cap_chunks, pad1;

    double freq_offset;
    double mu;
    double timing_freq;
    double afc_alpha;
    double p1r, p1i, p2r, p2i;
    double x40c, x40s;
    double fo_sum;
    double est_offset;
    uint32_t est_ties;
    uint32_t est_nsym;
    double energies[134];
    double est_poly[2 * OPV_OFFS_TERMS - 1];
    double est_power;

    uint64_t origin;
    uint64_t total_samples;
    uint64_t n_soft;
    uint32_t n_chunks;
    int32_t first_chunk_done;
    int32_t tail_done;
    int32_t overflow;
    int32_t stalled;
    uint32_t edge_ties;

    int32_t trk_state;
    int32_t trk_collecting;
    uint64_t trk_anchor;
    uint64_t trk_next;
    double trk_quality;
    int32_t trk_misses;
    int32_t trk_sync_ok;
    uint32_t n_frames;
    uint32_t n_events;
    uint32_t dec_from;

    uint32_t dbg_hw_id, dbg_xcc_id;
    uint64_t dbg_cycles, dbg_ticks;
};

#define OPV_TIE_SLOTS_MAX 512
#define OPV_TIE_PASSES_MAX 8
struct OpvTieSlot {
    uint32_t stream;
    uint32_t nsym;
    double poly[2 * OPV_OFFS_TERMS - 1];
    double power;
    double est;
    uint32_t ties;
    uint32_t pad;
    double energies[134];
    alignas(16) int16_t iq[2 * OPV_SPS * 1000];
};
struct OpvTieStage {
    uint32_t n;
    uint32_t listed;
    uint32_t beyond;
    uint32_t pad;
    OpvTieSlot slot[1];
};

#define OPV_MOVE_PIECE 32768u
struct OpvMove {
    const void* src;
    void* dst;
    uint32_t bytes;
    uint32_t pad;
};
struct OpvUnpackItem {
    OpvStream st;
    uint32_t stream;
    uint32_t live_first;
    uint32_t live_n;
    uint32_t pad;
};

struct OpvGlobalCfg {
    int32_t streaming;
    int32_t have_init_offset;
    double init_offset;
};
```

opv-cxx-demod_amd/csrc/opv_link.hip:

```cpp
#include <cstring>
#include <vector>

#include "opv_ctx.h"
#include "opv_stream_rules.h"

void link_launch(opv_ctx* c, uint64_t fr) {
    if (!c->link_on) return;
    k_frame_link<<<(unsigned)(fr * (uint64_t)c->n_streams), 64, 0, c->stream>>>(c->d_streams, c->d_link, c->cap_frames, (uint32_t)fr);
}

int link_clear(opv_ctx* c, int lo, int hi) {
    if (!c->d_link || hi <= lo) return OPV_OK;
    HIPCHK(hipMemsetAsync(c->d_link + (size_t)c->cap_frames * lo, 0, sizeof(opv_link) * c->cap_frames * (size_t)(hi - lo), c->stream));
    return OPV_OK;
}

extern "C" int opv_enable_link_report(opv_ctx* c, int enable) {
    if (!c) return fail(OPV_EINVAL, "null context");
    HIPCHK(hipSetDevice(c->cfg.device));
    if (enable && !c->link_on) {
        if (!c->d_link) {
            const hipError_t e = hipMalloc(&c->d_link, sizeof(opv_link) * c->cap_frames * (size_t)c->n_streams);
            if (e != hipSuccess) { c->d_link = nullptr; return alloc_failed(e, "hipMalloc", "opv_enable_link_report: the record ring"); }
        }
        if (int r = link_clear(c, 0, c->n_streams)) return r;
        HIPCHK(hipStreamSynchronize(c->stream));
        c->link_epoch = ~0u;
    }
    c->link_on = enable != 0;
    return OPV_OK;
}

extern "C" int opv_device_link(opv_ctx* c, const opv_link** d_link) {
    if (!c || !d_link) return fail(OPV_EINVAL, "null argument");
    if (!c->d_link) return fail(OPV_ESTATE, "opv_device_link: the link report was never enabled (opv_enable_link_report)");
    *d_link = c->d_link;
    return OPV_OK;
}

static int link_to_host(opv_ctx* c, int s, uint32_t first, uint32_t n, int32_t* met, opv_link* rec) {
    const RingRuns r = ring_runs(first, n, c->cap_frames);
    const size_t base = (size_t)c->cap_frames * s;
    bool have = false;
    if (int e = c->ensure_pools(&have)) return e;
    if (have) {
        if (c->link_epoch != c->mirror_epoch) {
            c->m_link.resize((size_t)c->cap_frames * c->n_streams);
            HIPCHK(hipMemcpyAsync(c->m_link.data(), c->d_link, c->m_link.size() * sizeof(opv_link), hipMemcpyDeviceToHost, c->stream));
            HIPCHK(hipStreamSynchronize(c->stream));
            c->link_epoch = c->mirror_epoch;
        }
        std::memcpy(met, c->m_metrics.data() + base + r.p0, sizeof(int32_t) * r.run0);
        std::memcpy(rec, c->m_link.data() + base + r.p0, sizeof(opv_link) * r.run0);
        if (r.run1) {
            std::memcpy(met + r.run0, c->m_metrics.data() + base, sizeof(int32_t) * r.run1);
            std::memcpy(rec + r.run0, c->m_link.data() + base, sizeof(opv_link) * r.run1);
        }
        return OPV_OK;
    }
    HIPCHK(hipMemcpyAsync(met, c->d_metrics + base + r.p0, sizeof(int32_t) * r.run0, hipMemcpyDeviceToHost, c->stream));
    HIPCHK(hipMemcpyAsync(rec, c->d_link + base + r.p0, sizeof(opv_link) * r.run0, hipMemcpyDeviceToHost, c->stream));
    if (r.run1) {
        HIPCHK(hipMemcpyAsync(met + r.run0, c->d_metrics + base, sizeof(int32_t) * r.run1, hipMemcpyDeviceToHost, c->stream));
        HIPCHK(hipMemcpyAsync(rec + r.run0, c->d_link + base, sizeof(opv_link) * r.run1, hipMemcpyDeviceToHost, c->stream));
    }
    HIPCHK(hipStreamSynchronize(c->stream));
    return OPV_OK;
}

extern "C" long opv_pop_frames_link(opv_ctx* c, int s, uint8_t* out, size_t cap, opv_frame_meta* meta, opv_link* link) {
    if (int r = check_stream(c, s)) return r;
    if (!link) return fail(OPV_EINVAL, "opv_pop_frames_link: null link");
    if (!c->link_on) return fail(OPV_ESTATE, "opv_pop_frames_link: the link report is off (opv_enable_link_report)");
    const uint32_t before = c->hs[s].popped;
    const long n = opv_pop_frames(c, s, out, cap, meta);
    if (n <= 0) return n;
    const uint32_t cnt = c->hs[s].popped - before;
    std::vector<int32_t> met(cnt);
    std::vector<opv_link> rec(cnt);
    if (int r = link_to_host(c, s, before, cnt, met.data(), rec.data())) return r;
    long w = 0;
    for (uint32_t k = 0; k < cnt && w < n; ++k)
        if (met[k] >= 0) link[w++] = rec[k];
    if (w != n) return fail(OPV_EHIP, "opv_pop_frames_link: the metrics ring disagrees with the frames handed out");
    return n;
}

extern "C" int opv_link_payloads(opv_ctx* c, const double* soft, size_t n, opv_link* out) {
    if (!c || !soft || !out) return fail(OPV_EINVAL, "null argument");
    if (n == 0 || n > 0x7FFFFFFFull) return fail(OPV_EINVAL, "opv_link_payloads: n_frames must be 1 .. 2^31 - 1");
    HIPCHK(hipSetDevice(c->cfg.device));
    double *d_soft = nullptr, *d_scale = nullptr;
    uint8_t* d_out = nullptr;
    int32_t* d_met = nullptr;
    opv_link* d_rec = nullptr;
    int rc = OPV_OK;
    auto chk = [&](hipError_t e, const char* w) { if (e != hipSuccess && rc == OPV_OK) rc = fail(OPV_EHIP, w, e); };
    chk(hipMalloc(&d_soft, sizeof(double) * OPV_CODED * n), "hipMalloc soft");
    chk(hipMalloc(&d_scale, sizeof(double) * n), "hipMalloc scales");
    chk(hipMalloc(&d_out, (size_t)OPV_FB * n), "hipMalloc frames");
    chk(hipMalloc(&d_met, sizeof(int32_t) * n), "hipMalloc metrics");
    chk(hipMalloc(&d_rec, sizeof(opv_link) * n), "hipMalloc records");
    if (rc == OPV_OK) {
        chk(hipMemcpyAsync(d_soft, soft, sizeof(double) * OPV_CODED * n, hipMemcpyHostToDevice, c->stream), "H2D soft");
        chk(hipMemsetAsync(d_out, 0, (size_t)OPV_FB * n, c->stream), "memset");
        k_payload_scale<<<(unsigned)((n + 63) / 64), 64, 0, c->stream>>>(d_soft, (uint32_t)n, d_scale);
        k_decode_payloads<<<(unsigned)((n + 1) / 2), 64, 0, c->stream>>>(d_soft, (uint32_t)n, d_scale, d_out, d_met, nullptr, nullptr, nullptr);
        k_link_payloads<<<(unsigned)n, 64, 0, c->stream>>>(d_soft, (uint32_t)n, d_scale, d_out, d_met, d_rec);
        chk(hipGetLastError(), "k_link_payloads launch");
        chk(hipMemcpyAsync(out, d_rec, sizeof(opv_link) * n, hipMemcpyDeviceToHost, c->stream), "D2H records");
        chk(hipStreamSynchronize(c->stream), "sync");
    }
    void* ptrs[] = {d_soft, d_scale, d_out, d_met, d_rec};
    for (void* p : ptrs) if (p) (void)hipFree(p);
    return rc;
}
```

opv-cxx-demod_amd/csrc/opv_migrate.hip:

```cpp
#include <climits>
#include <cstring>

#include "opv_ctx.h"
#include "opv_stream_rules.h"

namespace {
int mig_buffers(opv_ctx* c, size_t dev_bytes, size_t tab_bytes) {
    if (int r = c->mig.grow(dev_bytes, dev_bytes + dev_bytes / 4 + 65536, {c->stream}, "stream migration: device staging buffer")) return r;
    return c->mig_tab.grow(tab_bytes, tab_bytes + tab_bytes / 4 + 65536, {c->stream}, "stream migration: pinned table");
}

unsigned mig_grid(size_t items) { return (unsigned)(items < 1 ? 1 : items > 4096 ? 4096 : items); }

int mig_time(opv_ctx* c, bool end) {
    if (!c->timing) return OPV_OK;
    if (!end) { HIPCHK(hipEventRecord(c->ev[0], c->stream)); return OPV_OK; }
    for (int k = 1; k < 8; ++k) HIPCHK(hipEventRecord(c->ev[k], c->stream));
    c->timing_valid = true;
    return OPV_OK;
}

int plan_export(opv_ctx* c, int count, const int* streams, std::vector<BlobEntry>* ents, uint64_t* payload) {
    if (!c) return fail(OPV_EINVAL, "null context");
    if (count < 0 || (count > 0 && !streams)) return fail(OPV_EINVAL, "opv_export_streams: bad arguments");
    for (int i = 0; i < count; ++i)
        if (streams[i] < 0 || streams[i] >= c->n_streams) return fail(OPV_EINVAL, "opv_export_streams: stream index out of range");
    if (int r = settle_pushes(c)) return r;
    HIPCHK(hipStreamSynchronize(c->copy_stream));
    c->mirror_valid = false;
    if (int r = c->refresh()) return r;
    ents->assign((size_t)count, BlobEntry{});
    uint64_t total = 0;
    for (int i = 0; i < count; ++i) {
        const HostStream& h = c->hs[streams[i]];
        BlobEntry& e = (*ents)[i];
        OpvStream st = c->mirror[streams[i]];
        if (st.overflow) return fail(OPV_ESTATE, "opv_export_streams: the stream is in an error state (opv_pop_frames reports it)");
        if (h.soft_tapped) return fail(OPV_ESTATE, "opv_export_streams: the stream holds staged soft symbols (opv_tap_push_soft, a parity tap)");
        if (st.n_frames - h.popped > st.cap_frames) return fail(OPV_ESTATE, "opv_export_streams: more unpopped frames than the ring holds");
        const uint64_t keep = h.d_iq ? iq_keep(st.origin) : 0;
        uint64_t n_avail = h.d_iq ? h.n_avail : 0;
        e.last_round_avail = h.last_round_avail;
        iq_rebase(keep, &n_avail, &e.last_round_avail, &st);
        e.seg_n[SEG_IQ] = st.n_avail = n_avail;
        if (e.last_round_avail > st.n_avail) e.last_round_avail = st.n_avail;
        e.soft_first = soft_tail_first(st);
        e.seg_n[SEG_SOFT] = st.n_soft - e.soft_first;
        e.popped = h.popped;
        e.seg_n[SEG_FREC] = e.seg_n[SEG_FRAMES] = e.seg_n[SEG_METRICS] = e.seg_n[SEG_FSCALE] = st.n_frames - h.popped;
        e.events_popped = h.events_popped;
        e.events_dropped = h.events_dropped;
        if (st.n_events - e.events_popped > st.cap_events) {
            e.events_dropped += (st.n_events - e.events_popped) - st.cap_events;
            e.events_popped = st.n_events - st.cap_events;
        }
        e.events_first = e.events_popped;
        e.seg_n[SEG_EVENTS] = st.n_events - e.events_first;
        e.seg_n[SEG_CHUNKS] = st.n_chunks < st.cap_chunks ? st.n_chunks : st.cap_chunks;
        if (st.n_chunks - (uint32_t)e.seg_n[SEG_CHUNKS] < h.chunk_floor) e.seg_n[SEG_CHUNKS] = st.n_chunks - h.chunk_floor;
        e.chunks_first = st.n_chunks - (uint32_t)e.seg_n[SEG_CHUNKS];
        e.decoded = h.decoded;
        e.perfect = h.perfect;
        e.eof = h.eof;
        e.search_seen = h.search_seen ? 1 : 0;
        st.eof = h.eof;
        st.frames_popped = e.popped;
        st.events_popped = e.events_popped;
        st.iq = nullptr; st.soft = nullptr; st.frec = nullptr; st.events = nullptr; st.chunk_log = nullptr;
        st.frames = nullptr; st.metrics = nullptr; st.fscale = nullptr;
        e.st = st;
        e.off = total;
        uint64_t o = 0;
        for (int k = 0; k < SEG_N; ++k) { e.seg_off[k] = o; o += up16(e.seg_n[k] * kSegElem[k]); }
        e.len = o;
        total += o;
    }
    *payload = total;
    return OPV_OK;
}

}

extern "C" size_t opv_export_size(opv_ctx* c, int count, const int* streams) {
    std::vector<BlobEntry> ents;
    uint64_t payload = 0;
    if (plan_export(c, count, streams, &ents, &payload) != OPV_OK) return 0;
    return (size_t)(blob_payload_off(count) + payload);
}

extern "C" long opv_export_streams(opv_ctx* c, int count, const int* streams, void* blob, size_t cap) {
    std::vector<BlobEntry> ents;
    uint64_t payload = 0;
    if (int r = plan_export(c, count, streams, &ents, &payload)) return r;
    if (!blob) return fail(OPV_EINVAL, "opv_export_streams: null blob");
    BlobHeader h{};
    h.magic = kBlobMagic;
    h.version = kBlobVersion;
    h.sizeof_stream = sizeof(OpvStream);
    h.sizeof_header = sizeof(BlobHeader);
    h.sizeof_entry = sizeof(BlobEntry);
    h.streaming = c->cfg.streaming;
    h.coherent = c->cfg.coherent;
    h.have_init_offset = c->cfg.have_init_offset;
    h.init_offset_hz = c->cfg.have_init_offset ? c->cfg.init_offset_hz : 0.0;
    h.pll_bw_hz = c->cfg.coherent ? c->cfg.pll_bw_hz : 0.0;
    h.count = (uint32_t)count;
    h.payload_off = blob_payload_off(count);
    h.payload_bytes = payload;
    h.total_bytes = h.payload_off + payload;
    if (h.total_bytes > cap) return fail(OPV_ECAPACITY, "opv_export_streams: blob buffer too small (opv_export_size)");
    std::vector<OpvMove> mv;
    if (int r = mig_buffers(c, (size_t)payload, 0)) return r;
    for (int i = 0; i < count; ++i) {
        const BlobEntry& e = ents[i];
        const HostStream& hs = c->hs[streams[i]];
        const OpvStream& m = c->mirror[streams[i]];
        BlobSegment seg[SEG_N];
        blob_segments(e, m, (const char*)hs.d_iq + (e.st.iq_base - m.iq_base) * 4, seg);
        for (int k = 0; k < SEG_N; ++k) segment_moves(&mv, e, k, seg[k], c->mig.p + e.off, false);
    }
    if (int r = mig_buffers(c, (size_t)payload, mv.size() * sizeof(OpvMove))) return r;
    char* out = (char*)blob;
    std::memset(out, 0, (size_t)h.payload_off);
    std::memcpy(out, &h, sizeof h);
    if (count) std::memcpy(out + sizeof h, ents.data(), (size_t)count * sizeof(BlobEntry));
    if (payload) {
        std::memcpy(c->mig_tab.p, mv.data(), mv.size() * sizeof(OpvMove));
        void* d_tab = nullptr;
        HIPCHK(hipHostGetDevicePointer(&d_tab, c->mig_tab.p, 0));
        if (int r = mig_time(c, false)) return r;
        HIPCHK(hipMemsetAsync(c->mig.p, 0, (size_t)payload, c->stream));
        k_stream_pack<<<mig_grid(mv.size()), 256, 0, c->stream>>>((const OpvMove*)d_tab, (uint32_t)mv.size());
        HIPCHK(hipGetLastError());
        HIPCHK(hipMemcpyAsync(out + h.payload_off, c->mig.p, (size_t)payload, hipMemcpyDeviceToHost, c->stream));
        if (int r = mig_time(c, true)) return r;
        HIPCHK(hipStreamSynchronize(c->stream));
    }
    for (int i = 0; i < count; ++i) {
        const BlobEntry& e = ents[i];
        const char* met = out + h.payload_off + e.off + e.seg_off[SEG_METRICS];
        for (uint64_t k = 0; k < e.seg_n[SEG_METRICS]; ++k) {
            int32_t v;
            std::memcpy(&v, met + 4 * k, 4);
            if (v == INT32_MIN) return fail(OPV_ESTATE, "opv_export_streams: a released frame has not been decoded yet (call opv_process first)");
        }
    }
    return (long)h.total_bytes;
}

extern "C" int opv_blob_streams(const void* blob, size_t bytes) {
    BlobHeader h;
    if (const char* why = parse_blob(blob, bytes, &h, nullptr)) return fail(OPV_EINVAL, why);
    return (int)h.count;
}

extern "C" int opv_import_streams(opv_ctx* c, int count, const int* dst, const void* blob, size_t bytes) {
    if (!c) return fail(OPV_EINVAL, "null context");
    if (count < 0 || (count > 0 && !dst)) return fail(OPV_EINVAL, "opv_import_streams: bad arguments");
    BlobHeader h;
    std::vector<BlobEntry> ents;
    if (const char* why = parse_blob(blob, bytes, &h, &ents)) return fail(OPV_EINVAL, why);
    if ((uint32_t)count != h.count) return fail(OPV_EINVAL, "opv_import_streams: count differs from the streams in the blob (opv_blob_streams)");
    {
        std::vector<char> seen((size_t)c->n_streams, 0);
        for (int i = 0; i < count; ++i) {
            if (dst[i] < 0 || dst[i] >= c->n_streams) return fail(OPV_EINVAL, "opv_import_streams: destination stream index out of range");
            if (seen[dst[i]]) return fail(OPV_EINVAL, "opv_import_streams: a destination stream is named twice");
            seen[dst[i]] = 1;
        }
    }
    const opv_cfg& g = c->cfg;
    if (h.streaming != g.streaming || h.coherent != g.coherent || h.have_init_offset != g.have_init_offset ||
        (g.have_init_offset && h.init_offset_hz != g.init_offset_hz) || (g.coherent && h.pll_bw_hz != g.pll_bw_hz))
        return fail(OPV_EINVAL, "opv_import_streams: the blob was exported under another configuration (streaming / coherent / init_offset_hz / pll_bw_hz)");
    for (const BlobEntry& e : ents) {
        if (e.seg_n[SEG_IQ] > g.max_samples) return fail(OPV_ECAPACITY, "opv_import_streams: a stream's unconsumed IQ exceeds the destination's max_samples");
        if (e.seg_n[SEG_SOFT] > c->cap_soft) return fail(OPV_ECAPACITY, "opv_import_streams: a stream's soft-symbol tail exceeds the destination's ring");
        if (e.seg_n[SEG_FREC] > c->cap_frames) return fail(OPV_ECAPACITY, "opv_import_streams: more unpopped frames than the destination's frame_capacity");
    }
    if (count == 0) return OPV_OK;
    if (int r = settle_pushes(c)) return r;
    HIPCHK(hipStreamSynchronize(c->copy_stream));
    for (int i = 0; i < count; ++i) {
        if (ents[i].seg_n[SEG_IQ])
            if (int r = ensure_iq_buffer(c, c->hs[dst[i]], 0, "opv_import_streams: IQ buffer")) return r;
    }
    std::vector<OpvMove> mv;
    std::vector<OpvUnpackItem> items((size_t)count);
    if (int r = mig_buffers(c, (size_t)h.payload_bytes, 0)) return r;
    for (int i = 0; i < count; ++i) {
        const BlobEntry& e = ents[i];
        const HostStream& hs = c->hs[dst[i]];
        const OpvStream& ini = c->initial[dst[i]];
        OpvUnpackItem& it = items[i];
        std::memset(&it, 0, sizeof it);
        OpvStream& st = it.st;
        st = e.st;
        st.iq = hs.d_iq_owned;
        st.soft = ini.soft; st.cap_soft = ini.cap_soft;
        st.frec = ini.frec; st.events = ini.events; st.chunk_log = ini.chunk_log;
        st.frames = ini.frames; st.metrics = ini.metrics; st.fscale = ini.fscale;
        st.cap_frames = ini.cap_frames; st.cap_events = ini.cap_events; st.cap_chunks = ini.cap_chunks;
        it.stream = (uint32_t)dst[i];
        it.live_first = e.popped % ini.cap_frames;
        it.live_n = (uint32_t)e.seg_n[SEG_FREC];
        BlobSegment seg[SEG_N];
        blob_segments(e, st, hs.d_iq_owned, seg);
        for (int k = 0; k < SEG_N; ++k) segment_moves(&mv, e, k, seg[k], c->mig.p + e.off, true);
    }
    const size_t items_bytes = (items.size() * sizeof(OpvUnpackItem) + 15u) & ~(size_t)15u;
    if (int r = mig_buffers(c, (size_t)h.payload_bytes, items_bytes + mv.size() * sizeof(OpvMove))) return r;
    std::memcpy(c->mig_tab.p, items.data(), items.size() * sizeof(OpvUnpackItem));
    if (!mv.empty()) std::memcpy((char*)c->mig_tab.p + items_bytes, mv.data(), mv.size() * sizeof(OpvMove));
    void* d_tab = nullptr;
    HIPCHK(hipHostGetDevicePointer(&d_tab, c->mig_tab.p, 0));
    if (int r = mig_time(c, false)) return r;
    if (h.payload_bytes) HIPCHK(hipMemcpyAsync(c->mig.p, (const char*)blob + h.payload_off, (size_t)h.payload_bytes, hipMemcpyHostToDevice, c->stream));
    k_stream_unpack<<<mig_grid(items.size() + mv.size()), 256, 0, c->stream>>>(c->d_streams, c->d_counts, (const OpvUnpackItem*)d_tab, (uint32_t)items.size(),
                                                                             (const OpvMove*)((char*)d_tab + items_bytes), (uint32_t)mv.size());
    HIPCHK(hipGetLastError());
    if (int r = mig_time(c, true)) return r;
    for (int i = 0; i < count; ++i) {
        const BlobEntry& e = ents[i];
        HostStream n = reset_host_stream(c->hs[dst[i]]);
        n.n_avail = e.seg_n[SEG_IQ];
        n.eof = e.eof;
        n.dirty = true;
        n.search_seen = e.search_seen != 0;
        n.last_round_avail = e.last_round_avail;
        n.popped = e.popped;
        n.events_popped = e.events_popped;
        n.events_dropped = e.events_dropped;
        n.decoded = e.decoded;
        n.perfect = e.perfect;
        n.soft_floor = e.soft_first;
        n.iq_seen = true;
        n.chunk_floor = e.chunks_first + (uint32_t)(e.seg_n[SEG_CHUNKS] - (e.seg_n[SEG_CHUNKS] < c->cap_chunks ? e.seg_n[SEG_CHUNKS] : c->cap_chunks));
        c->hs[dst[i]] = n;
    }
    c->mirror_valid = false;
    c->maybe_stalled = true;
    for (int i = 0; i < count; ++i)
        if (int r = link_clear(c, dst[i], dst[i] + 1)) return r;
    HIPCHK(hipStreamSynchronize(c->stream));
    return OPV_OK;
}
```

opv-cxx-demod_amd/csrc/opv_stream_rules.cpp:

```cpp
#include "opv_stream_rules.h"

#include <cstring>

uint64_t soft_tail_first(const OpvStream& st) {
    uint64_t lo = st.trk_next;
    if (st.trk_state != OPV_HUNTING && st.trk_anchor + 1 < lo) lo = st.trk_anchor + 1;
    lo = lo >= 24 ? lo - 24 : 0;
    if (lo > st.n_soft) lo = st.n_soft;
    lo &= ~1ull;
    if (st.n_soft > st.cap_soft && lo < st.n_soft - st.cap_soft) lo = (st.n_soft - st.cap_soft + 1) & ~1ull;
    return lo;
}

const char* parse_blob(const void* blob, size_t bytes, BlobHeader* h, std::vector<BlobEntry>* ents) {
    if (!blob || bytes < sizeof(BlobHeader)) return "stream blob: missing or shorter than its header";
    std::memcpy(h, blob, sizeof *h);
    if (h->magic != kBlobMagic) return "stream blob: wrong magic";
    if (h->version != kBlobVersion || h->sizeof_stream != sizeof(OpvStream) || h->sizeof_header != sizeof(BlobHeader) || h->sizeof_entry != sizeof(BlobEntry))
        return "stream blob: written by another build of the library (format version / struct sizes differ)";
    if (h->total_bytes > bytes || h->total_bytes < sizeof(BlobHeader)) return "stream blob: truncated";
    if (h->count > 0x7FFFFFFFu || (uint64_t)h->count > (h->total_bytes - sizeof(BlobHeader)) / sizeof(BlobEntry)) return "stream blob: stream count does not fit the blob";
    const uint64_t dir_end = sizeof(BlobHeader) + (uint64_t)h->count * sizeof(BlobEntry);
    if ((h->payload_off & 15u) || h->payload_off < dir_end || h->payload_off > h->total_bytes || h->payload_bytes != h->total_bytes - h->payload_off)
        return "stream blob: payload offset / length out of range";
    if (!ents) return nullptr;
    ents->resize(h->count);
    if (h->count) std::memcpy(ents->data(), (const char*)blob + sizeof(BlobHeader), (size_t)h->count * sizeof(BlobEntry));
    for (const BlobEntry& e : *ents) {
        if ((e.off & 15u) || e.off > h->payload_bytes || e.len > h->payload_bytes - e.off) return "stream blob: a stream's payload lies outside the blob";
        for (int k = 0; k < SEG_N; ++k) {
            if (e.seg_n[k] >= (1ull << 31)) return "stream blob: segment length out of range";
            const uint64_t b = e.seg_n[k] * kSegElem[k];
            if ((e.seg_off[k] & 15u) || e.seg_off[k] > e.len || b > e.len - e.seg_off[k]) return "stream blob: a segment lies outside its stream's payload";
        }
        const OpvStream& st = e.st;
        const uint32_t nf = (uint32_t)e.seg_n[SEG_FREC];
        bool ok = e.seg_n[SEG_IQ] == st.n_avail && st.origin <= st.n_avail && st.overflow == 0;
        ok = ok && e.soft_first + e.seg_n[SEG_SOFT] == st.n_soft && (e.soft_first & 1u) == 0 && e.soft_first <= soft_tail_first(st) && st.trk_next <= st.n_soft;
        ok = ok && e.seg_n[SEG_FRAMES] == nf && e.seg_n[SEG_METRICS] == nf && e.seg_n[SEG_FSCALE] == nf && e.popped + nf == st.n_frames;
        ok = ok && e.events_first + (uint32_t)e.seg_n[SEG_EVENTS] == st.n_events && e.events_first == e.events_popped;
        ok = ok && e.chunks_first + (uint32_t)e.seg_n[SEG_CHUNKS] == st.n_chunks && e.last_round_avail <= st.n_avail;
        if (!ok) return "stream blob: a stream's indices contradict its segments";
    }
    return nullptr;
}

void blob_segments(const BlobEntry& e, const OpvStream& r, const void* iq, BlobSegment seg[SEG_N]) {
    seg[SEG_IQ] = {(char*)iq, e.seg_n[SEG_IQ], 0, e.seg_n[SEG_IQ], false};
    seg[SEG_SOFT] = {(char*)r.soft, r.cap_soft, e.soft_first, e.seg_n[SEG_SOFT], false};
    seg[SEG_FREC] = {(char*)r.frec, r.cap_frames, e.popped, e.seg_n[SEG_FREC], false};
    seg[SEG_FRAMES] = {(char*)r.frames, r.cap_frames, e.popped, e.seg_n[SEG_FRAMES], false};
    seg[SEG_METRICS] = {(char*)r.metrics, r.cap_frames, e.popped, e.seg_n[SEG_METRICS], false};
    seg[SEG_FSCALE] = {(char*)r.fscale, r.cap_frames, e.popped, e.seg_n[SEG_FSCALE], false};
    seg[SEG_EVENTS] = {(char*)r.events, r.cap_events, e.events_first, e.seg_n[SEG_EVENTS], true};
    seg[SEG_CHUNKS] = {(char*)r.chunk_log, r.cap_chunks, e.chunks_first, e.seg_n[SEG_CHUNKS], true};
}

void segment_moves(std::vector<OpvMove>* mv, const BlobEntry& e, int k, const BlobSegment& g, char* base, bool to_ring) {
    const uint64_t elem = kSegElem[k], n = g.lossy && g.n > g.cap ? g.cap : g.n, skip = g.n - n;
    if (n == 0) return;
    const RingRuns r = ring_runs(g.first + skip, n, g.cap);
    char* linear = base + e.seg_off[k] + skip * elem;
    const struct { uint64_t slot, bytes; } runs[2] = {{r.p0, r.run0 * elem}, {0, r.run1 * elem}};
    for (const auto& run : runs) {
        for (uint64_t o = 0; o < run.bytes; o += OPV_MOVE_PIECE) {
            const uint64_t b = run.bytes - o < OPV_MOVE_PIECE ? run.bytes - o : OPV_MOVE_PIECE;
            char* in_ring = g.ring + run.slot * elem + o;
            mv->push_back(to_ring ? OpvMove{linear + o, in_ring, (uint32_t)b, 0} : OpvMove{in_ring, linear + o, (uint32_t)b, 0});
        }
        linear += run.bytes;
    }
}
```

opv-cxx-demod_amd/csrc/opv_stream_rules.h:

```cpp
#pragma once
#include <stddef.h>
#include <stdint.h>

#include <vector>

#include "../../include/opv_demod.h"
#include "opv_device.h"

inline uint64_t iq_keep(uint64_t origin) { return origin >= 16 ? ((origin - 16) & ~3ull) : 0; }

inline void iq_rebase(uint64_t keep, uint64_t* n_avail, uint64_t* last_round_avail, OpvStream* st) {
    *n_avail -= keep;
    *last_round_avail = *last_round_avail > keep ? *last_round_avail - keep : 0;
    st->origin -= keep;
    st->n_avail -= keep;
    st->iq_base += keep;
}

struct RingRuns { uint64_t p0, run0, run1; };
inline RingRuns ring_runs(uint64_t first, uint64_t n, uint64_t cap) {
    const uint64_t p0 = first % cap, run0 = n < cap - p0 ? n : cap - p0;
    return {p0, run0, n - run0};
}

inline uint64_t soft_keep(const OpvStream& st) {
    uint64_t keep = st.trk_next >= 24 ? st.trk_next - 24 : 0;
    if (st.trk_state != OPV_HUNTING && st.trk_anchor < keep) keep = st.trk_anchor;
    return keep;
}

struct LaunchShape { uint32_t slices, grid; };
inline LaunchShape table_launch(uint32_t items, uint32_t most, uint32_t unit, uint32_t grid_cap) {
    uint32_t slices = items >= 1024 ? 1 : (1024 + items - 1) / items;
    const uint32_t by_size = most / (256u * unit);
    if (slices > by_size) slices = by_size ? by_size : 1;
    const uint32_t grid = items * slices;
    return {slices, grid > grid_cap ? grid_cap : grid};
}

constexpr uint64_t kBlobMagic = 0x31424f4c4256504full;
constexpr uint32_t kBlobVersion = 1;
enum { SEG_IQ, SEG_SOFT, SEG_FREC, SEG_FRAMES, SEG_METRICS, SEG_FSCALE, SEG_EVENTS, SEG_CHUNKS, SEG_N };
constexpr uint64_t kSegElem[SEG_N] = {4, sizeof(double), sizeof(OpvFrameRec), OPV_FB, sizeof(int32_t), sizeof(double), sizeof(OpvEventRec), 5 * sizeof(double)};

struct BlobHeader {
    uint64_t magic;
    uint32_t version, sizeof_stream, sizeof_header, sizeof_entry;
    int32_t streaming, coherent, have_init_offset;
    uint32_t count;
    double init_offset_hz, pll_bw_hz;
    uint64_t total_bytes, payload_off, payload_bytes;
};
struct BlobEntry {
    uint64_t off, len;
    uint64_t seg_off[SEG_N];
    uint64_t seg_n[SEG_N];
    uint64_t soft_first;
    uint32_t events_first, chunks_first;
    uint32_t popped, events_popped, events_dropped;
    int32_t decoded, perfect, eof, search_seen, pad;
    uint64_t last_round_avail;
    OpvStream st;
};

inline uint64_t up16(uint64_t v) { return (v + 15u) & ~15ull; }
inline uint64_t blob_payload_off(int count) { return (sizeof(BlobHeader) + (uint64_t)count * sizeof(BlobEntry) + 255u) & ~255ull; }

uint64_t soft_tail_first(const OpvStream& st);

const char* parse_blob(const void* blob, size_t bytes, BlobHeader* h, std::vector<BlobEntry>* ents);

struct BlobSegment { char* ring; uint64_t cap, first, n; bool lossy; };
void blob_segments(const BlobEntry& e, const OpvStream& rings, const void* iq, BlobSegment seg[SEG_N]);

void segment_moves(std::vector<OpvMove>* mv, const BlobEntry& e, int k, const BlobSegment& g, char* base, bool to_ring);
```

Baseline: 9314 Msamples/s.

## Split each round so decode of the bulk overlaps the frontend tail on a side stream

When a streaming round has many fresh chunks, the frontend first runs on all but a short tail of samples, then sync-track, scale, decode and link run on that prefix on a second HIP stream. Meanwhile the frontend finishes the tail on the main stream. A shortened consumer pass then handles the remainder, so the serial frontend→decoder dependency is partly hidden by concurrency. It adds snapshot tracker fields and split cap/restore kernels, changes the debug counters to accumulate, and retunes the nop padding at the symbol-loop top. The cost is extra launches, events and correctness risk at the split boundary.

```diff
diff --git a/opv-cxx-demod_amd/csrc/k_frontend.hip b/opv-cxx-demod_amd/csrc/k_frontend.hip
--- a/opv-cxx-demod_amd/csrc/k_frontend.hip
+++ b/opv-cxx-demod_amd/csrc/k_frontend.hip
@@ -215,8 +215,8 @@
     uint32_t edge_ties = uni(st.edge_ties);
     const uint64_t cap_soft = st.cap_soft;
     if (cap_soft > (1ull << 28)) overflow = 1;
-    uint64_t soft_keep = st.trk_next >= 24 ? st.trk_next - 24 : 0;
-    if (st.trk_state != 0 && st.trk_anchor < soft_keep) soft_keep = st.trk_anchor;
+    uint64_t soft_keep = st.fe_trk_next >= 24 ? st.fe_trk_next - 24 : 0;
+    if (st.fe_trk_state != 0 && st.fe_trk_anchor < soft_keep) soft_keep = st.fe_trk_anchor;
     const uint32_t soft_bmask = (uint32_t)(cap_soft * 8u - 1u) & ~7u;
     gbyte* const soft_base = (gbyte*)(((uint64_t)uni((uint32_t)((uint64_t)st.soft >> 32)) << 32) | uni((uint32_t)(uint64_t)st.soft));
     const gbyte* iq_bytes = (const gbyte*)st.iq;
@@ -557,7 +557,8 @@
                 uint32_t more = uni(housekeeping(pos, NoAdvance{}));
                 if (F64 && overflow != 0) break;
                 fetch(pos, false);
-                if constexpr (F64) asm volatile("; opv_symbol_loop_top\n\ts_nop 0\n\ts_nop 0\n\ts_nop 0\n\ts_nop 0\n\ts_nop 0\n\ts_nop 0");
+                if constexpr (F64) asm volatile("; opv_symbol_loop_top\n\ts_nop 0\n\ts_nop 0\n\ts_nop 0\n\ts_nop 0");
+                else if constexpr (WPB == 1) asm volatile("; opv_symbol_loop_top_at_24\n\ts_nop 0\n\ts_nop 0\n\ts_nop 0\n\ts_nop 0\n\ts_nop 0\n\ts_nop 0\n\ts_nop 0\n\ts_nop 0\n\ts_nop 0\n\ts_nop 0\n\ts_nop 0\n\ts_nop 0");
                 while (more >= 4u) {
                     for (uint32_t quads = more >> 2; quads != 0u; --quads) {
                         sym(TagSteady{}, Slot0{}, qq, qp);
@@ -615,8 +616,8 @@
         asm volatile("s_getreg_b32 %0, hwreg(HW_REG_HW_ID)" : "=s"(hw));
         asm volatile("s_getreg_b32 %0, hwreg(HW_REG_XCC_ID)" : "=s"(xcc));
         st.dbg_hw_id = hw; st.dbg_xcc_id = xcc;
-        st.dbg_cycles = __builtin_amdgcn_s_memtime() - dbg_t0;
-        st.dbg_ticks = __builtin_amdgcn_s_memrealtime() - dbg_r0;
+        st.dbg_cycles += __builtin_amdgcn_s_memtime() - dbg_t0;
+        st.dbg_ticks += __builtin_amdgcn_s_memrealtime() - dbg_r0;
     }
 }
 
diff --git a/opv-cxx-demod_amd/csrc/k_frontend_rows.h b/opv-cxx-demod_amd/csrc/k_frontend_rows.h
--- a/opv-cxx-demod_amd/csrc/k_frontend_rows.h
+++ b/opv-cxx-demod_amd/csrc/k_frontend_rows.h
@@ -33,8 +33,8 @@
         eof = st.eof;
         cap_soft = st.cap_soft;
         if (cap_soft > (1ull << 28)) overflow = 1;
-        soft_keep = st.trk_next >= 24 ? st.trk_next - 24 : 0;
-        if (st.trk_state != 0 && st.trk_anchor < soft_keep) soft_keep = st.trk_anchor;
+        soft_keep = st.fe_trk_next >= 24 ? st.fe_trk_next - 24 : 0;
+        if (st.fe_trk_state != 0 && st.fe_trk_anchor < soft_keep) soft_keep = st.fe_trk_anchor;
         soft_bmask = (uint32_t)(cap_soft * 8u - 1u) & ~7u;
         soft_base = (gbyte*)st.soft;
         iq_bytes = (const gbyte*)st.iq;
@@ -57,8 +57,8 @@
         asm volatile("s_getreg_b32 %0, hwreg(HW_REG_HW_ID)" : "=s"(hw));
         asm volatile("s_getreg_b32 %0, hwreg(HW_REG_XCC_ID)" : "=s"(xcc));
         st.dbg_hw_id = hw; st.dbg_xcc_id = xcc;
-        st.dbg_cycles = __builtin_amdgcn_s_memtime() - dbg_t0;
-        st.dbg_ticks = __builtin_amdgcn_s_memrealtime() - dbg_r0;
+        st.dbg_cycles += __builtin_amdgcn_s_memtime() - dbg_t0;
+        st.dbg_ticks += __builtin_amdgcn_s_memrealtime() - dbg_r0;
     }
 
     __device__ __forceinline__ void flush_soft() {
diff --git a/opv-cxx-demod_amd/csrc/k_sync_track.hip b/opv-cxx-demod_amd/csrc/k_sync_track.hip
--- a/opv-cxx-demod_amd/csrc/k_sync_track.hip
+++ b/opv-cxx-demod_amd/csrc/k_sync_track.hip
@@ -26,18 +26,18 @@
 
 }
 
-extern "C" __global__ __launch_bounds__(64) void k_sync_track(OpvStream* __restrict__ streams) {
+extern "C" __global__ __launch_bounds__(64) void k_sync_track(OpvStream* __restrict__ streams, uint32_t pass_a) {
     OpvStream& st = streams[blockIdx.x];
     const int lane = threadIdx.x;
     const double* __restrict__ soft = st.soft;
     const uint32_t mask = (uint32_t)(st.cap_soft - 1);
-    const uint64_t n = st.n_soft;
+    const uint64_t n = pass_a ? st.trk_bound : st.n_soft;
 
     int state = st.trk_state, collecting = st.trk_collecting, misses = st.trk_misses;
     uint64_t anchor = st.trk_anchor, next = st.trk_next;
     double quality = st.trk_quality;
     uint32_t n_frames = st.n_frames, n_events = st.n_events;
-    int overflow = st.overflow;
+    const int overflow = pass_a ? n == ~0ull : st.overflow;
     if (lane == 0) st.dec_from = n_frames;
 
     auto event = [&](int kind, int count, uint64_t sym, double corr, double raw) {
@@ -143,6 +143,6 @@
         st.trk_state = state; st.trk_collecting = collecting; st.trk_misses = misses;
         st.trk_anchor = anchor; st.trk_next = next; st.trk_quality = quality;
         st.n_frames = n_frames; st.n_events = n_events; st.trk_sync_ok = sync_ok;
-        st.stalled |= stalled;
+        if (!pass_a) st.stalled |= stalled;
     }
 }
diff --git a/opv-cxx-demod_amd/csrc/opv_capi.hip b/opv-cxx-demod_amd/csrc/opv_capi.hip
--- a/opv-cxx-demod_amd/csrc/opv_capi.hip
+++ b/opv-cxx-demod_amd/csrc/opv_capi.hip
@@ -29,6 +29,32 @@
         }
         streams[i].frames_popped = in[i].frames_popped;
         streams[i].events_popped = in[i].events_popped;
+        streams[i].fe_trk_next = streams[i].trk_next;
+        streams[i].fe_trk_anchor = streams[i].trk_anchor;
+        streams[i].fe_trk_state = streams[i].trk_state;
+        streams[i].dbg_cycles = 0;
+        streams[i].dbg_ticks = 0;
+    }
+}
+
+__global__ void k_split_cap(OpvStream* streams, const StreamIn* in, int n) {
+    const int i = blockIdx.x * blockDim.x + threadIdx.x;
+    if (i < n && in[i].dirty) {
+        uint64_t cap = in[i].n_avail_a;
+        if (cap < streams[i].origin) cap = streams[i].origin;
+        if (cap < streams[i].n_avail) streams[i].n_avail = cap;
+        streams[i].eof = 0;
+    }
+}
+
+__global__ void k_split_restore(OpvStream* streams, const StreamIn* in, int n) {
+    const int i = blockIdx.x * blockDim.x + threadIdx.x;
+    if (i < n) {
+        if (in[i].dirty) {
+            streams[i].n_avail = in[i].n_avail;
+            streams[i].eof = in[i].eof;
+        }
+        streams[i].trk_bound = streams[i].overflow ? ~0ull : streams[i].n_soft;
     }
 }
 
@@ -138,6 +164,7 @@
     c->push_gather = !std::getenv("OPV_PUSH_NO_GATHER");
     if (const char* e = std::getenv("OPV_PUSH_GATHER_BLOCKS")) { const int v = atoi(e); if (v > 0) c->push_gather_blocks = (uint32_t)v; }
     c->rb_fp64_ring = !std::getenv("OPV_FRONTEND_INT16_RING");
+    c->split = split_rule_from_env(std::getenv("OPV_PROCESS_SPLIT"));
     {
         hipFuncAttributes fa;
         HIPCHK_C(hipFuncGetAttributes(&fa, (const void*)k_msk_frontend_rb));
@@ -201,6 +228,11 @@
     if (c->tie.stage) (void)hipHostFree(c->tie.stage);
     if (c->push_ev) (void)hipEventDestroy(c->push_ev);
     if (c->done_ev) (void)hipEventDestroy(c->done_ev);
+    if (c->side_stream) { (void)hipStreamSynchronize(c->side_stream); (void)hipStreamDestroy(c->side_stream); }
+    if (c->split_a) (void)hipEventDestroy(c->split_a);
+    if (c->split_done) (void)hipEventDestroy(c->split_done);
+    for (auto& e : c->ev2)
+        if (e) (void)hipEventDestroy(e);
     if (c->copy_stream) (void)hipStreamDestroy(c->copy_stream);
     for (auto& h : c->hs) { (void)hipFree(h.d_iq_owned); (void)hipFree(h.d_iq_alt); }
     for (auto& e : c->ev)
@@ -234,7 +266,7 @@
     c->search_now.clear();
     for (int i = 0; i < S; ++i) {
         const HostStream& h = c->hs[i];
-        in[i] = {h.d_iq, h.n_avail, h.eof, h.dirty ? 1 : 0, h.popped, h.events_popped};
+        in[i] = {h.d_iq, h.n_avail, h.eof, h.dirty ? 1 : 0, h.popped, h.events_popped, h.n_avail};
         if (h.dirty) any = true;
         if (!h.search_seen && (c->cfg.streaming ? h.n_avail >= (uint64_t)OPV_CHUNK : h.eof != 0)) c->search_now.push_back(i);
         const uint64_t fresh = h.n_avail - h.last_round_avail;
@@ -242,7 +274,7 @@
         if (h.tap_fresh) any = true;
         if (h.tap_fresh > max_tapped) max_tapped = h.tap_fresh;
     }
-    if (!any && c->maybe_stalled && c->round_no > 0 && hipEventQuery(c->done_ev) == hipSuccess)
+    if (c->maybe_stalled && c->stall_from_round && c->round_no > 0 && hipEventQuery(c->done_ev) == hipSuccess)
         c->maybe_stalled = c->h_stall[(c->round_no - 1) % opv_ctx::kInSlots] != 0;
     if (!any && !c->maybe_stalled) return OPV_OK;
     uint64_t fr = max_new / (uint64_t)(OPV_FSYMS * 38);
@@ -250,8 +282,30 @@
     fr += 4;
     if (fr > c->cap_frames) fr = c->cap_frames;
     if (fr * (uint64_t)S > 0x7FFFFFFFull) return fail(OPV_EINVAL, "opv_process: streams x frames per round exceeds the grid limit");
+    c->split_in.resize(S);
+    c->split_cap.resize(S);
+    for (int i = 0; i < S; ++i) {
+        const HostStream& h = c->hs[i];
+        c->split_in[i] = {h.n_avail, h.last_round_avail, h.tap_fresh, h.fed_since + (h.n_avail - h.last_round_avail) + 40u * h.tap_fresh,
+                          h.frames_base, h.popped, h.eof, 0};
+    }
+    uint64_t tail_most = 0;
+    const SplitRound sr{c->cfg.streaming, c->cfg.coherent, c->maybe_stalled ? 1 : 0, c->cap_frames, c->cap_soft};
+    const uint32_t tail = process_split(c->split, sr, c->split_in.data(), S, c->split_cap.data(), &tail_most);
+    if (tail) {
+        if (!c->side_stream) HIPCHK(hipStreamCreateWithFlags(&c->side_stream, hipStreamNonBlocking));
+        if (!c->split_a) HIPCHK(hipEventCreateWithFlags(&c->split_a, hipEventDisableTiming));
+        if (!c->split_done) HIPCHK(hipEventCreateWithFlags(&c->split_done, hipEventDisableTiming));
+    }
+    if (tail && c->timing)
+        for (auto& e : c->ev2)
+            if (!e) HIPCHK(hipEventCreate(&e));
+    uint64_t fr_b = (tail_most + 2u * (uint64_t)OPV_CHUNK) / (uint64_t)(OPV_FSYMS * 38) + 4;
+    if (fr_b > fr) fr_b = fr;
+    for (int i = 0; i < S; ++i) in[i].n_avail_a = c->split_cap[i];
     for (int i = 0; i < S; ++i) {
         HostStream& h = c->hs[i];
+        h.fed_since = c->split_in[i].fed;
         h.last_round_avail = h.n_avail;
         h.dirty = false;
         h.tap_fresh = 0;
@@ -259,6 +313,7 @@
     for (int i : c->search_now) c->hs[i].search_seen = true;
     c->mirror_valid = false;
     c->maybe_stalled = true;
+    c->stall_from_round = true;
     c->h_stall[slot] = 0;
     if (c->push_pending) HIPCHK(hipStreamWaitEvent(c->stream, c->push_ev, 0));
     HIPCHK(hipMemcpyAsync(c->d_in, in, sizeof(StreamIn) * S, hipMemcpyHostToDevice, c->stream));
@@ -287,40 +342,65 @@
             k_tie_apply<<<K, 192, 0, c->stream>>>(c->d_streams, c->tie.stage, K, S);
         }
     }
+    auto frontend = [&]() {
+        const bool x4 = c->frontend == 4 || (c->frontend == 0 && S >= kFrontendX4MinStreams);
+        if (c->cfg.coherent && !c->cfg.streaming) {
+            const double wn = c->cfg.pll_bw_hz * 2.0 * M_PI, zeta = 0.707, fsym = 2168000.0 / 40.0;
+            c->last_frontend = "k_coherent_frontend";
+            k_coherent_frontend<<<S, 64, 0, c->stream>>>(c->d_streams, 2.0 * zeta * wn / fsym, wn * wn / (fsym * fsym));
+        }
+        else if (c->frontend == 16 || (c->frontend == 0 && S > kFrontendX16MinStreams)) {
+            if (S > kFrontendX16Wg8MinStreams) { c->last_frontend = "k_msk_frontend_x16_wg8"; k_msk_frontend_x16_wg8<<<(S + 127) / 128, 512, 0, c->stream>>>(c->d_streams, g, S); }
+            else if (S > 16) { c->last_frontend = "k_msk_frontend_x16_wg4"; k_msk_frontend_x16_wg4<<<(S + 63) / 64, 256, 0, c->stream>>>(c->d_streams, g, S); }
+            else { c->last_frontend = "k_msk_frontend_x16"; k_msk_frontend_x16<<<1, 64, 0, c->stream>>>(c->d_streams, g, S); }
+        }
+        else if (x4) {
+            c->last_frontend = "k_msk_frontend_x4_wg4";
+            k_msk_frontend_x4_wg4<<<(S + 15) / 16, 256, 0, c->stream>>>(c->d_streams, g, S);
+        }
+        else if (S > kFrontendWg4MinStreams) {
+            c->last_frontend = "k_msk_frontend_rb_wg4";
+            k_msk_frontend_rb_wg4<<<(S + 3) / 4, 256, 0, c->stream>>>(c->d_streams, g, S);
+        } else if (c->rb_fp64_ring && S <= c->n_cu) {
+            c->last_frontend = "k_msk_frontend_rb";
+            k_msk_frontend_rb<<<S, 128, OPV_RB_LDS_F64, c->stream>>>(c->d_streams, g, S);
+        } else {
+            c->last_frontend = "k_msk_frontend_rb";
+            k_msk_frontend_rb<<<S, 64, OPV_RB_LDS_I16, c->stream>>>(c->d_streams, g, S);
+        }
+    };
+    auto consumers = [&](hipStream_t q, uint64_t frames, uint32_t pass_a, hipEvent_t* e) -> int {
+        if (e) HIPCHK(hipEventRecord(e[0], q));
+        k_sync_track<<<S, 64, 0, q>>>(c->d_streams, pass_a);
+        if (e) { HIPCHK(hipEventRecord(e[1], q)); HIPCHK(hipEventRecord(e[2], q)); }
+        if (frames * (uint64_t)S <= kScaleWaveMaxFrames) k_frame_scale_wave<<<(unsigned)(frames * (uint64_t)S), 64, 0, q>>>(c->d_streams, (uint32_t)frames);
+        else k_frame_scale<<<(unsigned)((frames * (uint64_t)S + 63) / 64), 64, 0, q>>>(c->d_streams, (uint32_t)frames, (uint32_t)S);
+        k_frame_decode<<<(unsigned)(((frames + 1) / 2) * (uint64_t)S), 64, 0, q>>>(c->d_streams, (uint32_t)((frames + 1) / 2));
+        if (e) HIPCHK(hipEventRecord(e[3], q));
+        link_launch(c, frames, q);
+        return OPV_OK;
+    };
     if (tm) HIPCHK(hipEventRecord(c->ev[2], c->stream));
-    const bool x4 = c->frontend == 4 || (c->frontend == 0 && S >= kFrontendX4MinStreams);
-    if (c->cfg.coherent && !c->cfg.streaming) {
-        const double wn = c->cfg.pll_bw_hz * 2.0 * M_PI, zeta = 0.707, fsym = 2168000.0 / 40.0;
-        c->last_frontend = "k_coherent_frontend";
-        k_coherent_frontend<<<S, 64, 0, c->stream>>>(c->d_streams, 2.0 * zeta * wn / fsym, wn * wn / (fsym * fsym));
-    }
-    else if (c->frontend == 16 || (c->frontend == 0 && S > kFrontendX16MinStreams)) {
-        if (S > kFrontendX16Wg8MinStreams) { c->last_frontend = "k_msk_frontend_x16_wg8"; k_msk_frontend_x16_wg8<<<(S + 127) / 128, 512, 0, c->stream>>>(c->d_streams, g, S); }
-        else if (S > 16) { c->last_frontend = "k_msk_frontend_x16_wg4"; k_msk_frontend_x16_wg4<<<(S + 63) / 64, 256, 0, c->stream>>>(c->d_streams, g, S); }
-        else { c->last_frontend = "k_msk_frontend_x16"; k_msk_frontend_x16<<<1, 64, 0, c->stream>>>(c->d_streams, g, S); }
-    }
-    else if (x4) {
-        c->last_frontend = "k_msk_frontend_x4_wg4";
-        k_msk_frontend_x4_wg4<<<(S + 15) / 16, 256, 0, c->stream>>>(c->d_streams, g, S);
-    }
-    else if (S > kFrontendWg4MinStreams) {
-        c->last_frontend = "k_msk_frontend_rb_wg4";
-        k_msk_frontend_rb_wg4<<<(S + 3) / 4, 256, 0, c->stream>>>(c->d_streams, g, S);
-    } else if (c->rb_fp64_ring && S <= c->n_cu) {
-        c->last_frontend = "k_msk_frontend_rb";
-        k_msk_frontend_rb<<<S, 128, OPV_RB_LDS_F64, c->stream>>>(c->d_streams, g, S);
+    if (tail) {
+        k_split_cap<<<(S + 63) / 64, 64, 0, c->stream>>>(c->d_streams, c->d_in, S);
+        frontend();
+        k_split_restore<<<(S + 63) / 64, 64, 0, c->stream>>>(c->d_streams, c->d_in, S);
+        if (tm) HIPCHK(hipEventRecord(c->ev[3], c->stream));
+        HIPCHK(hipEventRecord(c->split_a, c->stream));
+        HIPCHK(hipStreamWaitEvent(c->side_stream, c->split_a, 0));
+        if (int r = consumers(c->side_stream, fr, 1u, tm ? c->ev2 + 2 : nullptr)) return r;
+        HIPCHK(hipEventRecord(c->split_done, c->side_stream));
+        if (tm) HIPCHK(hipEventRecord(c->ev2[0], c->stream));
+        frontend();
+        if (tm) HIPCHK(hipEventRecord(c->ev2[1], c->stream));
+        HIPCHK(hipStreamWaitEvent(c->stream, c->split_done, 0));
+        if (int r = consumers(c->stream, fr_b, 0u, tm ? c->ev + 4 : nullptr)) return r;
     } else {
-        c->last_frontend = "k_msk_frontend_rb";
-        k_msk_frontend_rb<<<S, 64, OPV_RB_LDS_I16, c->stream>>>(c->d_streams, g, S);
-    }
-    if (tm) { HIPCHK(hipEventRecord(c->ev[3], c->stream)); HIPCHK(hipEventRecord(c->ev[4], c->stream)); }
-    k_sync_track<<<S, 64, 0, c->stream>>>(c->d_streams);
-    if (tm) { HIPCHK(hipEventRecord(c->ev[5], c->stream)); HIPCHK(hipEventRecord(c->ev[6], c->stream)); }
-    if (fr * (uint64_t)S <= kScaleWaveMaxFrames) k_frame_scale_wave<<<(unsigned)(fr * (uint64_t)S), 64, 0, c->stream>>>(c->d_streams, (uint32_t)fr);
-    else k_frame_scale<<<(unsigned)((fr * (uint64_t)S + 63) / 64), 64, 0, c->stream>>>(c->d_streams, (uint32_t)fr, (uint32_t)S);
-    k_frame_decode<<<(unsigned)(((fr + 1) / 2) * (uint64_t)S), 64, 0, c->stream>>>(c->d_streams, (uint32_t)((fr + 1) / 2));
-    if (tm) { HIPCHK(hipEventRecord(c->ev[7], c->stream)); c->timing_valid = true; }
-    link_launch(c, fr);
+        frontend();
+        if (tm) HIPCHK(hipEventRecord(c->ev[3], c->stream));
+        if (int r = consumers(c->stream, fr, 0u, tm ? c->ev + 4 : nullptr)) return r;
+    }
+    if (tm) { c->timing_valid = true; c->timing_split = tail != 0; }
     k_collect_counts<<<(S + 63) / 64, 64, 0, c->stream>>>(c->d_streams, c->d_counts, S, c->h_stall + slot);
     HIPCHK(hipEventRecord(c->done_ev, c->stream));
     HIPCHK(hipGetLastError());
@@ -375,6 +455,13 @@
     if (!c->timing_valid) return fail(OPV_ESTATE, "no timed opv_process yet (opv_enable_timing first)");
     HIPCHK(hipStreamSynchronize(c->stream));
     for (int k = 0; k < 4; ++k) HIPCHK(hipEventElapsedTime(&ms[k], c->ev[2 * k], c->ev[2 * k + 1]));
+    if (c->timing_split) {
+        for (int k = 0; k < 3; ++k) {
+            float t = 0.f;
+            HIPCHK(hipEventElapsedTime(&t, c->ev2[2 * k], c->ev2[2 * k + 1]));
+            ms[k + 1] += t;
+        }
+    }
     return OPV_OK;
 }
 
diff --git a/opv-cxx-demod_amd/csrc/opv_ctx.h b/opv-cxx-demod_amd/csrc/opv_ctx.h
--- a/opv-cxx-demod_amd/csrc/opv_ctx.h
+++ b/opv-cxx-demod_amd/csrc/opv_ctx.h
@@ -8,6 +8,7 @@
 
 #include "../../include/opv_demod.h"
 #include "opv_device.h"
+#include "opv_stream_rules.h"
 #include "opv_wb_internal.h"
 
 extern "C" __global__ void k_offset_search(OpvStream*, OpvGlobalCfg, const double*, uint32_t*);
@@ -20,7 +21,7 @@
 extern "C" __global__ void k_msk_frontend_x16_wg4(OpvStream*, OpvGlobalCfg, int);
 extern "C" __global__ void k_msk_frontend_x16_wg8(OpvStream*, OpvGlobalCfg, int);
 extern "C" __global__ void k_coherent_frontend(OpvStream*, double, double);
-extern "C" __global__ void k_sync_track(OpvStream*);
+extern "C" __global__ void k_sync_track(OpvStream*, uint32_t);
 extern "C" __global__ void k_frame_scale(OpvStream*, uint32_t, uint32_t);
 extern "C" __global__ void k_frame_scale_wave(OpvStream*, uint32_t);
 extern "C" __global__ void k_frame_decode(OpvStream*, uint32_t);
@@ -81,6 +82,7 @@
     int32_t eof;
     int32_t dirty;
     uint32_t frames_popped, events_popped;
+    uint64_t n_avail_a;
 };
 
 struct HostStream {
@@ -103,6 +105,8 @@
     bool iq_seen = false;
     bool soft_tapped = false;
     uint64_t tap_fresh = 0;
+    uint32_t frames_base = 0;
+    uint64_t fed_since = 0;
 };
 
 inline HostStream reset_host_stream(const HostStream& h) {
@@ -178,6 +182,14 @@
     bool timing = false;
     bool timing_valid = false;
     hipEvent_t ev[8] = {};
+    SplitRule split = kSplitDefault;
+    hipStream_t side_stream = nullptr;
+    hipEvent_t split_a = nullptr, split_done = nullptr;
+    hipEvent_t ev2[6] = {};
+    bool timing_split = false;
+    bool stall_from_round = false;
+    std::vector<SplitStream> split_in;
+    std::vector<uint64_t> split_cap;
 
     static constexpr size_t kPoolMirrorMax = 64u << 20;
     std::vector<uint8_t> m_frames;
@@ -197,6 +209,10 @@
         ++mirror_epoch;
         maybe_stalled = false;
         for (const OpvStream& m : mirror) maybe_stalled |= m.stalled != 0;
+        for (int i = 0; i < n_streams; ++i) {
+            hs[i].frames_base = mirror[i].n_frames;
+            hs[i].fed_since = mirror[i].n_avail > mirror[i].origin ? mirror[i].n_avail - mirror[i].origin : 0;
+        }
         return OPV_OK;
     }
     size_t pool_bytes() const {
@@ -246,7 +262,7 @@
     return OPV_OK;
 }
 
-void link_launch(opv_ctx* c, uint64_t fr);
+void link_launch(opv_ctx* c, uint64_t fr, hipStream_t q);
 int link_clear(opv_ctx* c, int lo, int hi);
 bool opv_tx_libm_flat_tops_as_assumed();
 int opv_tx_prepare_run(opv_ctx* c, size_t nsym);
diff --git a/opv-cxx-demod_amd/csrc/opv_device.h b/opv-cxx-demod_amd/csrc/opv_device.h
--- a/opv-cxx-demod_amd/csrc/opv_device.h
+++ b/opv-cxx-demod_amd/csrc/opv_device.h
@@ -85,9 +85,14 @@
     uint32_t n_events;
     uint32_t dec_from;
 
+    int32_t fe_trk_state, pad2;
+    uint64_t fe_trk_anchor, fe_trk_next;
+    uint64_t trk_bound;
+
     uint32_t dbg_hw_id, dbg_xcc_id;
     uint64_t dbg_cycles, dbg_ticks;
 };
+
 
 #define OPV_TIE_SLOTS_MAX 512
 #define OPV_TIE_PASSES_MAX 8
diff --git a/opv-cxx-demod_amd/csrc/opv_link.hip b/opv-cxx-demod_amd/csrc/opv_link.hip
--- a/opv-cxx-demod_amd/csrc/opv_link.hip
+++ b/opv-cxx-demod_amd/csrc/opv_link.hip
@@ -4,9 +4,9 @@
 #include "opv_ctx.h"
 #include "opv_stream_rules.h"
 
-void link_launch(opv_ctx* c, uint64_t fr) {
+void link_launch(opv_ctx* c, uint64_t fr, hipStream_t q) {
     if (!c->link_on) return;
-    k_frame_link<<<(unsigned)(fr * (uint64_t)c->n_streams), 64, 0, c->stream>>>(c->d_streams, c->d_link, c->cap_frames, (uint32_t)fr);
+    k_frame_link<<<(unsigned)(fr * (uint64_t)c->n_streams), 64, 0, q>>>(c->d_streams, c->d_link, c->cap_frames, (uint32_t)fr);
 }
 
 int link_clear(opv_ctx* c, int lo, int hi) {
diff --git a/opv-cxx-demod_amd/csrc/opv_migrate.hip b/opv-cxx-demod_amd/csrc/opv_migrate.hip
--- a/opv-cxx-demod_amd/csrc/opv_migrate.hip
+++ b/opv-cxx-demod_amd/csrc/opv_migrate.hip
@@ -17,6 +17,7 @@
     if (!end) { HIPCHK(hipEventRecord(c->ev[0], c->stream)); return OPV_OK; }
     for (int k = 1; k < 8; ++k) HIPCHK(hipEventRecord(c->ev[k], c->stream));
     c->timing_valid = true;
+    c->timing_split = false;
     return OPV_OK;
 }
 
@@ -235,11 +236,14 @@
         n.perfect = e.perfect;
         n.soft_floor = e.soft_first;
         n.iq_seen = true;
+        n.frames_base = e.st.n_frames;
+        n.fed_since = e.st.n_avail > e.st.origin ? e.st.n_avail - e.st.origin : 0;
         n.chunk_floor = e.chunks_first + (uint32_t)(e.seg_n[SEG_CHUNKS] - (e.seg_n[SEG_CHUNKS] < c->cap_chunks ? e.seg_n[SEG_CHUNKS] : c->cap_chunks));
         c->hs[dst[i]] = n;
     }
     c->mirror_valid = false;
     c->maybe_stalled = true;
+    c->stall_from_round = false;
     for (int i = 0; i < count; ++i)
         if (int r = link_clear(c, dst[i], dst[i] + 1)) return r;
     HIPCHK(hipStreamSynchronize(c->stream));
diff --git a/opv-cxx-demod_amd/csrc/opv_stream_rules.cpp b/opv-cxx-demod_amd/csrc/opv_stream_rules.cpp
--- a/opv-cxx-demod_amd/csrc/opv_stream_rules.cpp
+++ b/opv-cxx-demod_amd/csrc/opv_stream_rules.cpp
@@ -1,5 +1,6 @@
 #include "opv_stream_rules.h"
 
+#include <cstdlib>
 #include <cstring>
 
 uint64_t soft_tail_first(const OpvStream& st) {
@@ -10,6 +11,51 @@
     lo &= ~1ull;
     if (st.n_soft > st.cap_soft && lo < st.n_soft - st.cap_soft) lo = (st.n_soft - st.cap_soft + 1) & ~1ull;
     return lo;
+}
+
+uint32_t process_split(const SplitRule& rule, const SplitRound& round, const SplitStream* s, int n, uint64_t* cap_a, uint64_t* tail_most) {
+    for (int i = 0; i < n; ++i) cap_a[i] = s[i].n_avail;
+    *tail_most = 0;
+    if (!rule.enabled || rule.min_calls == 0 || !round.streaming || round.coherent || round.stall_possible) return 0;
+    uint64_t most_calls = 0;
+    for (int i = 0; i < n; ++i) {
+        if (s[i].tapped) return 0;
+        const uint64_t fresh = s[i].n_avail >= s[i].last_round_avail ? s[i].n_avail - s[i].last_round_avail : 0;
+        if (fresh / OPV_CHUNK > most_calls) most_calls = fresh / OPV_CHUNK;
+        const uint64_t pending = fresh + OPV_CHUNK;
+        if (pending / 38u + 2u * (pending / OPV_CHUNK + 1u) + OPV_FSYMS + OPV_SYNC_BITS > round.cap_soft) return 0;
+        if (frames_upper(s[i].frames_base, s[i].fed) > (uint64_t)s[i].popped + round.cap_frames) return 0;
+    }
+    if (most_calls < rule.min_calls) return 0;
+    const uint64_t tail = rule.tail_calls ? rule.tail_calls : (most_calls + 31u) / 32u;
+    if (tail >= most_calls) return 0;
+    const uint64_t tail_samples = tail * (uint64_t)OPV_CHUNK;
+    for (int i = 0; i < n; ++i) {
+        uint64_t cap = s[i].n_avail > tail_samples ? s[i].n_avail - tail_samples : 0;
+        if (cap < s[i].last_round_avail) cap = s[i].last_round_avail;
+        if (cap > s[i].n_avail) cap = s[i].n_avail;
+        cap_a[i] = cap;
+        if (s[i].n_avail - cap > *tail_most) *tail_most = s[i].n_avail - cap;
+    }
+    return (uint32_t)tail;
+}
+
+SplitRule split_rule_from_env(const char* text) {
+    SplitRule r = kSplitDefault;
+    if (!text) return r;
+    char* end = nullptr;
+    const unsigned long long a = std::strtoull(text, &end, 10);
+    if (end == text) return r;
+    if (*end == '\0') {
+        if (a == 0) r.enabled = 0;
+        return r;
+    }
+    if (*end != ',') return r;
+    const char* second = end + 1;
+    const unsigned long long b = std::strtoull(second, &end, 10);
+    if (end == second || *end != '\0') return r;
+    if (a > 0 && b > 0 && a <= 0xFFFFFFFFull && b <= 0xFFFFFFFFull) { r.min_calls = (uint32_t)a; r.tail_calls = (uint32_t)b; }
+    return r;
 }
 
 const char* parse_blob(const void* blob, size_t bytes, BlobHeader* h, std::vector<BlobEntry>* ents) {
diff --git a/opv-cxx-demod_amd/csrc/opv_stream_rules.h b/opv-cxx-demod_amd/csrc/opv_stream_rules.h
--- a/opv-cxx-demod_amd/csrc/opv_stream_rules.h
+++ b/opv-cxx-demod_amd/csrc/opv_stream_rules.h
@@ -38,6 +38,33 @@
     return {slices, grid > grid_cap ? grid_cap : grid};
 }
 
+struct SplitRule {
+    int32_t enabled;
+    uint32_t min_calls;
+    uint32_t tail_calls;
+};
+constexpr SplitRule kSplitDefault = {1, 64, 0};
+struct SplitRound {
+    int32_t streaming, coherent;
+    int32_t stall_possible;
+    uint32_t cap_frames;
+    uint64_t cap_soft;
+};
+struct SplitStream {
+    uint64_t n_avail;
+    uint64_t last_round_avail;
+    uint64_t tapped;
+    uint64_t fed;
+    uint32_t frames_base;
+    uint32_t popped;
+    int32_t eof, pad;
+};
+inline uint64_t frames_upper(uint64_t frames_base, uint64_t fed) {
+    return frames_base + (fed / 39u + fed / OPV_CHUNK + 2u) / OPV_FSYMS + 2u;
+}
+uint32_t process_split(const SplitRule& rule, const SplitRound& round, const SplitStream* s, int n, uint64_t* cap_a, uint64_t* tail_most);
+SplitRule split_rule_from_env(const char* text);
+
 constexpr uint64_t kBlobMagic = 0x31424f4c4256504full;
 constexpr uint32_t kBlobVersion = 1;
 enum { SEG_IQ, SEG_SOFT, SEG_FREC, SEG_FRAMES, SEG_METRICS, SEG_FSCALE, SEG_EVENTS, SEG_CHUNKS, SEG_N };
```

New measurement: 9358 Msamples/s (median of 6 runs). Within noise of the previous version (+0.5%).
